# zdebruine/singlet

Hardware: AMD Instinct MI355X
Metric: ALS iterations/sec (1M cells x 30k genes, 5% nnz, k=50) (higher is better)
Workload: dtype f64

## Files before the change

singlet_amd/csrc/gen_acc_tiled.py:

```python
#!/usr/bin/env python3
import os
import sys

NS = 8
ER = [64 + i for i in range(NS)]
EX = [72 + 2 * i for i in range(NS)]
AD = [88 + j for j in range(8)]
W = [96 + 4 * j for j in range(8)]
ACC = 128
S_RP, S_XP, S_NS, S_ACC = 84, 86, 88, 91
S_TP = 92
TAB0, TAB1 = 52, 68
S_END = 100


def r2(b):
    return f"v[{b}:{b + 1}]"


class Gen:

    def __init__(self, pair, pf=0):
        self.L = []
        self.lab = 0
        self.pair = pair
        self.pf = pf

    def A(self, s):
        self.L.append(s)

    def label(self, stem):
        self.lab += 1
        return f".Ltiled_{stem}_{self.lab}_%="

    def text(self):
        return " \\\n".join(f'    "{ins}\\n\\t"' for ins in self.L)

    def refill(self, i):
        if self.pair:
            st, sub = i >> 1, i & 1
            ro, xo, lap_r = 256 * st + 64 * sub, 512 * st + 128 * sub, 128 * NS
        else:
            ro, xo, lap_r = 256 * i, 512 * i, 256 * NS
        A = self.A
        A(f"global_load_dword v{ER[i]}, %[voff4], s[{S_RP}:{S_RP + 1}] offset:{ro}")
        A(f"global_load_dwordx2 {r2(EX[i])}, %[voff8], s[{S_XP}:{S_XP + 1}] offset:{xo}")
        if i == NS - 1:
            A(f"s_add_u32 s{S_RP}, s{S_RP}, {lap_r}")
            A(f"s_addc_u32 s{S_RP + 1}, s{S_RP + 1}, 0")
            A(f"s_add_u32 s{S_XP}, s{S_XP}, {2 * lap_r}")
            A(f"s_addc_u32 s{S_XP + 1}, s{S_XP + 1}, 0")

    def addrs(self, slot, o):
        for j in range(8):
            self.A(f"v_add_u32_dpp v{AD[j]}, v{ER[slot]}, %[lane16] row_newbcast:{8 * o + j} row_mask:0xf bank_mask:0xf")

    def octet(self, d, o, reads):
        A = self.A
        x = EX[d]
        for g in range(2):
            gi = 4 * d + 2 * o + g
            A(f"s_bfe_u32 m0, s{TAB0 + gi // 2}, {hex((16 * (gi & 1)) | (16 << 16))}")
            A(f"s_waitcnt lgkmcnt({4 if reads else 4 - 4 * g})")
            for j in range(4 * g, 4 * g + 4):
                bc = f"row_newbcast:{8 * o + j} row_mask:0xf bank_mask:0xf"
                A(f"v_fmac_f64_dpp {r2(ACC)}, {r2(x)}, {r2(W[j])} {bc}")
                A(f"v_fmac_f64_dpp {r2(ACC + 2)}, {r2(x)}, {r2(W[j] + 2)} {bc}")
                if reads:
                    A(f"ds_read_b128 v[{W[j]}:{W[j] + 3}], v{AD[j]}")

    def wrap(self):
        A = self.A
        A("s_waitcnt lgkmcnt(0)")
        for w in range(8):
            A(f"s_mov_b64 s[{TAB0 + 2 * w}:{TAB0 + 2 * w + 1}], s[{TAB1 + 2 * w}:{TAB1 + 2 * w + 1}]")
        A(f"s_load_dwordx16 s[{TAB1}:{TAB1 + 15}], s[{S_TP}:{S_TP + 1}], 0x0")
        A(f"s_add_u32 s{S_TP}, s{S_TP}, 64")
        A(f"s_addc_u32 s{S_TP + 1}, s{S_TP + 1}, 0")
        if self.pf:
            A("s_mov_b32 m0, 0")
            A("v_lshlrev_b32 v63, 1, %[pfl]")
            A(f"global_load_dword v63, v63, s[{S_XP}:{S_XP + 1}]")
            A(f"global_load_dword v63, %[pfl], s[{S_RP}:{S_RP + 1}]")

    def body(self, d, L_body, L_last):
        A = self.A
        dn = (d + 1) % NS
        A(f"{L_body[d]}:")
        A("s_mov_b32 m0, 0")
        self.addrs(d, 1)
        self.octet(d, 0, True)
        A("s_mov_b32 m0, 0")
        A(f"s_waitcnt vmcnt({2 * (NS - 2) + (2 if (self.pf and d != NS - 1) else 0)})")
        self.addrs(dn, 0)
        self.octet(d, 1, True)
        self.refill(d)
        if d == NS - 1:
            self.wrap()
        A(f"s_sub_u32 s{S_NS}, s{S_NS}, 1")
        A(f"s_cbranch_scc1 {L_last[dn]}")
        if d == NS - 1:
            A(f"s_branch {L_body[0]}")

    def last(self, d, L_last, L_end):
        A = self.A
        A(f"{L_last[d]}:")
        A("s_mov_b32 m0, 0")
        self.addrs(d, 1)
        self.octet(d, 0, True)
        self.octet(d, 1, False)
        self.refill(d)
        A(f"s_mov_b32 %[phase], {(d + 1) % NS}")
        A(f"s_branch {L_end}")

    def chunk(self):
        A = self.A
        L_body = [self.label(f"b{d}") for d in range(NS)]
        L_pro = [self.label(f"p{d}") for d in range(NS)]
        L_last = [self.label(f"last{d}") for d in range(NS)]
        L_end = self.label("end")
        A(f"s_mov_b64 s[{S_RP}:{S_RP + 1}], %[rp]")
        A(f"s_mov_b64 s[{S_XP}:{S_XP + 1}], %[xp]")
        A(f"s_sub_u32 s{S_NS}, %[ns], 2")
        A(f"s_lshl_b32 s{S_ACC}, %[phase], 3")
        A(f"s_mov_b64 s[{S_TP}:{S_TP + 1}], %[tp]")
        A(f"s_sub_u32 s{S_TP}, s{S_TP}, s{S_ACC}")
        A(f"s_subb_u32 s{S_TP + 1}, s{S_TP + 1}, 0")
        A(f"s_load_dwordx16 s[{TAB0}:{TAB0 + 15}], s[{S_TP}:{S_TP + 1}], 0x0")
        A(f"s_load_dwordx16 s[{TAB1}:{TAB1 + 15}], s[{S_TP}:{S_TP + 1}], 0x40")
        A(f"s_add_u32 s{S_TP}, s{S_TP}, 128")
        A(f"s_addc_u32 s{S_TP + 1}, s{S_TP + 1}, 0")
        A(f"s_mov_b32 s{S_ACC}, 0")
        A(f"s_set_gpr_idx_on s{S_ACC}, 0")
        A("s_mov_b32 m0, 0")
        for d in range(1, NS):
            A(f"s_cmp_eq_u32 %[phase], {d}")
            A(f"s_cbranch_scc1 {L_pro[d]}")
        for d in range(NS):
            A(f"{L_pro[d]}:")
            A(f"s_waitcnt vmcnt({2 * (NS - 1)})")
            self.addrs(d, 0)
            for j in range(8):
                A(f"ds_read_b128 v[{W[j]}:{W[j] + 3}], v{AD[j]}")
            A("s_waitcnt lgkmcnt(0)")
            A(f"s_cmp_eq_u32 %[ns], 1")
            A(f"s_cbranch_scc1 {L_last[d]}")
            A(f"s_branch {L_body[d]}")
        for d in range(NS):
            self.body(d, L_body, L_last)
        for d in range(NS):
            self.last(d, L_last, L_end)
        A(f"{L_end}:")
        A("s_waitcnt lgkmcnt(0)")
        A("s_mov_b32 m0, 0")
        A("s_set_gpr_idx_off")
        A(f"s_mov_b64 %[rp], s[{S_RP}:{S_RP + 1}]")
        A(f"s_mov_b64 %[xp], s[{S_XP}:{S_XP + 1}]")

    def ring_fill(self):
        A = self.A
        A(f"s_mov_b64 s[{S_RP}:{S_RP + 1}], %[rp]")
        A(f"s_mov_b64 s[{S_XP}:{S_XP + 1}], %[xp]")
        for i in range(NS):
            self.refill(i)
        A(f"s_mov_b64 %[rp], s[{S_RP}:{S_RP + 1}]")
        A(f"s_mov_b64 %[xp], s[{S_XP}:{S_XP + 1}]")


def main():
    pf = int(os.environ.get("SGL_GEN_PF", "0"))
    out = ["// generated by gen_acc_tiled.py -- do not edit", "#pragma once"]
    g = Gen(pair=False)
    for c in range(128):
        g.A(f"v_mov_b32 v{ACC + c}, 0")
    out.append(f"#define ACC_TILED_ZERO_ASM \\\n{g.text()}")
    out.append("#define ACC_TILED_CLOBBERS " + ", ".join([f'"s{r}"' for r in range(83, S_END)] + ['"memory"', '"scc"']))
    for tag, pair in (("2", True), ("4", False)):
        g = Gen(pair)
        g.ring_fill()
        out.append("")
        out.append(f"#define ACC_TILED{tag}_RING_FILL_ASM \\\n{g.text()}")
        g = Gen(pair, pf)
        g.chunk()
        out.append("")
        out.append(f"#define ACC_TILED{tag}_CHUNK_ASM \\\n{g.text()}")
    tclob = [f'"s{r}"' for r in range(TAB0, S_END)] + ['"memory"', '"scc"'] + (['"v63"'] if pf else [])
    out.append("#define ACC_TILED_CHUNK_CLOBBERS " + ", ".join(tclob))
    out.append(f"#define ACC_TILED_PF_LAPS {pf}")
    sys.stdout.write("\n".join(out) + "\n")


if __name__ == "__main__":
    main()
```

singlet_amd/csrc/kernels_tiled.hip:

```cpp
#include "sgl_internal.h"
#include <hipcub/hipcub.hpp>
#include <stdlib.h>
#include <utility>
#include <type_traits>

#define TILED_NW 8
#define TILED_CW 64
#define TILED_NP 32
#define TILED_LDS_BYTES (160 * 1024 - 512)
#define TILED_SLACK 4096

__device__ __forceinline__ int64_t tiled_slot_col(const int32_t* __restrict__ perm, int64_t ncol, int64_t wb, int h, int p, int nsl) {
    const int64_t pos = wb * (TILED_NP * nsl) + nsl * p + h;
    if (pos >= ncol) return -1;
    return perm ? (int64_t)perm[pos] : pos;
}

__device__ __forceinline__ int tiled_ranges_of(int64_t wb, int R, int64_t tail_wg0, int tail_R) {
    return (tail_R > 1 && tail_wg0 >= 0 && wb / TILED_NW >= tail_wg0) ? tail_R : R;
}
__device__ __forceinline__ int tiled_range_end(int b, int T, int NB, int nr) {
    const int t = b >> 1;
    const int y = (int)(((int64_t)(t + 1) * nr - 1) / T);
    const int b1 = 2 * (int)(((int64_t)(y + 1) * T) / nr);
    return b1 < NB ? b1 : NB;
}

__global__ __launch_bounds__(256) void tiled_count_kernel(const int64_t* __restrict__ seg, const int32_t* __restrict__ perm, int64_t ncol,
                                                          int T, int NB, int64_t nwb, int R, int64_t tail_wg0, int tail_R,
                                                          uint8_t* __restrict__ cnt, uint16_t* __restrict__ ahead,
                                                          int64_t* __restrict__ chunk_entries, int nsl) {
    const int lane = threadIdx.x & 63, p = lane & 31;
    const int64_t wb = ((int64_t)blockIdx.x * blockDim.x + threadIdx.x) >> 6;
    if (wb >= nwb) return;
    const int gps = 16 / nsl;
    int64_t col[4];
    for (int h = 0; h < 4; ++h) col[h] = h < nsl ? tiled_slot_col(perm, ncol, wb, h, p, nsl) : -1;
    const int nr = tiled_ranges_of(wb, R, tail_wg0, tail_R);
    for (int b0 = 0; b0 < NB;) {
        const int b1 = tiled_range_end(b0, T, NB, nr);
        int64_t pos[4];
        for (int h = 0; h < 4; ++h) pos[h] = col[h] >= 0 ? seg[(int64_t)b0 * ncol + col[h]] : 0;
        for (int b = b0; b < b1; ++b) {
            const int hi = b + 2 < b1 ? b + 2 : b1;
            int64_t must = 0, avail = 0, ew[4];
            for (int h = 0; h < 4; ++h) {
                ew[h] = 0;
                if (col[h] >= 0) {
                    const int64_t eb = seg[(int64_t)(b + 1) * ncol + col[h]];
                    ew[h] = seg[(int64_t)hi * ncol + col[h]];
                    must = eb - pos[h] > must ? eb - pos[h] : must;
                    avail = ew[h] - pos[h] > avail ? ew[h] - pos[h] : avail;
                }
            }
            int g = (int)((must + 3) >> 2);
            const int cap = (int)((avail + 3) >> 2) - g;
            int tot = g;
            for (int o = 16; o > 0; o >>= 1) tot += __shfl_xor(tot, o, 32);
            const int rem = (gps - (tot & (gps - 1))) & (gps - 1);
            int suf = cap;
            for (int o = 1; o < 32; o <<= 1) {
                const int v = __shfl_down(suf, o, 32);
                if (p + o < 32) suf += v;
            }
            const int above = suf - cap;
            int extra = rem - above < cap ? rem - above : cap;
            if (extra < 0) extra = 0;
            const int all = __shfl(suf, 0, 32);
            if (p == TILED_NP - 1 && rem > all) extra += rem - all;
            g += extra;
            const int64_t u = wb * NB + b;
            if (lane < 32) {
                cnt[u * TILED_NP + p] = (uint8_t)g;
                for (int h = 0; h < nsl; ++h)
                    ahead[u * (TILED_NP * nsl) + nsl * p + h] = col[h] >= 0 ? (uint16_t)(pos[h] - seg[(int64_t)b * ncol + col[h]]) : (uint16_t)0;
            }
            if (lane == 0) chunk_entries[u] = (int64_t)(tot + rem) * 4 * nsl;
            for (int h = 0; h < 4; ++h) pos[h] += (4 * (int64_t)g < ew[h] - pos[h]) ? 4 * (int64_t)g : ew[h] - pos[h];
        }
        b0 = b1;
    }
}

__global__ __launch_bounds__(256) void tiled_fill_kernel(const double* __restrict__ x, const int32_t* __restrict__ idx,
                                                         const int64_t* __restrict__ seg, const int32_t* __restrict__ perm,
                                                         int64_t ncol, int T, int NB, int64_t nwb, int R, int64_t tail_wg0, int tail_R,
                                                         int D, int row_bytes, const uint8_t* __restrict__ cnt,
                                                         const uint16_t* __restrict__ ahead, const int64_t* __restrict__ cstart,
                                                         uint32_t* __restrict__ sroff, double* __restrict__ sx,
                                                         int masked, uint64_t seed, SglDiv inv_density, int mask_t,
                                                         int64_t col_off, int64_t row_off, int nsl) {
    const int lane = threadIdx.x & 63;
    const int eps = 64 / nsl, eps_sh = nsl == 4 ? 4 : 5;
    const int64_t gw = ((int64_t)blockIdx.x * blockDim.x + threadIdx.x) >> 6;
    const int64_t nw = ((int64_t)gridDim.x * blockDim.x) >> 6;
    for (int64_t u = gw; u < nwb * NB; u += nw) {
        const int64_t wb = u / NB;
        const int b = (int)(u - wb * NB);
        const int b1 = tiled_range_end(b, T, NB, tiled_ranges_of(wb, R, tail_wg0, tail_R));
        const int hi = b + 2 < b1 ? b + 2 : b1;
        const int64_t c0 = cstart[u];
        int P = 0;
        for (int p = 0; p < TILED_NP; ++p) {
            const int n4 = 4 * (int)cnt[u * TILED_NP + p];
            if (n4 == 0) continue;
            for (int h = 0; h < nsl; ++h) {
                const int64_t col = tiled_slot_col(perm, ncol, wb, h, p, nsl);
                int64_t a = 0, e = 0;
                if (col >= 0) {
                    a = seg[(int64_t)b * ncol + col] + ahead[u * (TILED_NP * nsl) + nsl * p + h];
                    e = seg[(int64_t)hi * ncol + col];
                }
                for (int q = lane; q < n4; q += 64) {
                    uint32_t ro = 0;
                    double xv = 0.0;
                    if (a + q < e) {
                        const int32_t r = idx[a + q];
                        const int blk = r >= (b + 1) * D ? b + 1 : b;
                        ro = (uint32_t)((blk & 1) * D + (r - blk * D)) * (uint32_t)row_bytes;
                        xv = x[a + q];
                        if (masked) {
                            const uint64_t gc = (uint64_t)(col + col_off), gr = (uint64_t)(r + row_off);
                            if (mask_t ? sgl_draw(seed, gr, gc, inv_density) : sgl_draw(seed, gc, gr, inv_density)) xv = 0.0;
                        }
                    }
                    const int pos = P + q;
                    const int64_t dst = c0 + (int64_t)(pos >> eps_sh) * 64 + h * eps + (pos & (eps - 1));
                    if (sroff != nullptr) sroff[dst] = ro;
                    sx[dst] = xv;
                }
            }
            P += n4;
        }
    }
}

__global__ __launch_bounds__(256) void tiled_gtab_kernel(const uint8_t* __restrict__ cnt, const int64_t* __restrict__ cstart,
                                                         int64_t nchunks, int nsl, uint16_t* __restrict__ gtab) {
    const int lane = threadIdx.x & 63;
    const int64_t gw = ((int64_t)blockIdx.x * blockDim.x + threadIdx.x) >> 6;
    const int64_t nw = ((int64_t)gridDim.x * blockDim.x) >> 6;
    for (int64_t u = gw; u < nchunks; u += nw) {
        int64_t g0 = cstart[u] / (4 * nsl);
        for (int p = 0; p < TILED_NP; ++p) {
            const int n = (int)cnt[u * TILED_NP + p];
            for (int q = lane; q < n; q += 64) gtab[g0 + q] = (uint16_t)(0x8000u | (unsigned)(4 * p));
            g0 += n;
        }
    }
}

template <typename T_>
static int t_alloc(T_** p, size_t count) {
    *p = nullptr;
    if (count == 0) count = 1;
    hipError_t e = sgl_pool_malloc((void**)p, count * sizeof(T_));
    if (e != hipSuccess) {
        (void)hipGetLastError();
        sgl_set_error("hipMalloc of %zu bytes failed: %s", count * sizeof(T_), hipGetErrorString(e));
        return SGL_ENOMEM;
    }
    return SGL_OK;
}

template <typename T_>
static int t_reserve(T_** p, size_t* cap, size_t count) {
    if (*p != nullptr && *cap >= count) return SGL_OK;
    if (*p) (void)sgl_pool_free(*p);
    *p = nullptr;
    *cap = 0;
    const size_t want = count + count / 32 + 64;
    SGLCHK(t_alloc(p, want));
    *cap = want;
    return SGL_OK;
}

void sgl_tiled_free(DevTiled& S) {
    if (S.seg) (void)sgl_pool_free(S.seg);
    if (S.perm) (void)sgl_pool_free(S.perm);
    if (S.roff) (void)sgl_pool_free(S.roff);
    if (S.x) (void)sgl_pool_free(S.x);
    if (S.cstart) (void)sgl_pool_free(S.cstart);
    if (S.cnt) (void)sgl_pool_free(S.cnt);
    if (S.ahead) (void)sgl_pool_free(S.ahead);
    if (S.gtab) (void)sgl_pool_free(S.gtab);
    if (S.part) (void)sgl_pool_free(S.part);
    if (S.xm) (void)sgl_pool_free(S.xm);
    S = DevTiled();
}

static bool tiled_sort_columns() {
    const char* e = getenv("SGL_TILED_SORT");
    return !(e && *e == '0');
}

__global__ void tiled_col_keys_kernel(const int64_t* __restrict__ p, int64_t ncol, uint32_t* __restrict__ keys, int32_t* __restrict__ iota) {
    for (int64_t c = (int64_t)blockIdx.x * blockDim.x + threadIdx.x; c < ncol; c += (int64_t)gridDim.x * blockDim.x) {
        keys[c] = (uint32_t)(p[c + 1] - p[c]);
        iota[c] = (int32_t)c;
    }
}

static int tiled_build_perm(sgl_ctx* c, const DevCSC& M, DevTiled& S) {
    hipStream_t s = c->stream;
    const int64_t n = M.ncol;
    SGLCHK(t_reserve(&S.perm, &S.cap_perm, (size_t)n));
    uint32_t *keys = nullptr, *keys_out = nullptr;
    int32_t* iota = nullptr;
    void* tmp = nullptr;
    int rc = t_alloc(&keys, (size_t)n);
    if (rc == SGL_OK) rc = t_alloc(&keys_out, (size_t)n);
    if (rc == SGL_OK) rc = t_alloc(&iota, (size_t)n);
    if (rc == SGL_OK && n > 0) {
        const int64_t blocks = std::min<int64_t>((n + 255) / 256, 4096);
        tiled_col_keys_kernel<<<dim3((unsigned)blocks), dim3(256), 0, s>>>(M.p, n, keys, iota);
        size_t tmp_bytes = 0;
        if (hipcub::DeviceRadixSort::SortPairsDescending(nullptr, tmp_bytes, keys, keys_out, iota, S.perm, n, 0, 32, s) != hipSuccess) rc = SGL_EHIP;
        if (rc == SGL_OK && sgl_pool_malloc(&tmp, tmp_bytes ? tmp_bytes : 1) != hipSuccess) { (void)hipGetLastError(); rc = SGL_ENOMEM; }
        if (rc == SGL_OK && hipcub::DeviceRadixSort::SortPairsDescending(tmp, tmp_bytes, keys, keys_out, iota, S.perm, n, 0, 32, s) != hipSuccess) rc = SGL_EHIP;
    }
    static_assert(TILED_CW == 64, "pair layout: 64 columns per wave");
    std::vector<uint32_t> top_v((size_t)TILED_NW * TILED_CW * 2);
    uint32_t* top = top_v.data();
    const int64_t ntop = std::min<int64_t>(n, (int64_t)top_v.size());
    if (rc == SGL_OK && ntop > 0 && hipMemcpyAsync(top, keys_out, sizeof(uint32_t) * (size_t)ntop, hipMemcpyDeviceToHost, s) != hipSuccess) rc = SGL_EHIP;
    const hipError_t e = hipStreamSynchronize(s);
    if (rc == SGL_OK && e == hipSuccess) {
        int64_t tn = 0, tn2 = 0;
        for (int64_t q = 0; q < ntop; ++q) {
            if (q < TILED_NW * TILED_CW) tn += top[q];
            tn2 += top[q];
        }
        S.top_share = M.nnz > 0 ? (double)tn / (double)M.nnz : 0.0;
        S.top_share4 = M.nnz > 0 ? (double)tn2 / (double)M.nnz : 0.0;
    }
    if (keys) (void)sgl_pool_free(keys);
    if (keys_out) (void)sgl_pool_free(keys_out);
    if (iota) (void)sgl_pool_free(iota);
    if (tmp) (void)sgl_pool_free(tmp);
    if (rc == SGL_OK && e != hipSuccess) rc = SGL_EHIP;
    if (rc != SGL_OK) { sgl_set_error("tiled build: sorting the columns by their non-zero count failed"); return rc; }
    S.perm_nnz = M.nnz;
    return SGL_OK;
}

void sgl_trace_setup(const char* what);

int sgl_tiled_build(sgl_ctx* c, const DevCSC& M, int k, DevTiled& S) {
    hipStream_t s = c->stream;
    const int nsl = (k <= 32 && !getenv("SGL_TILED_NO_QUAD")) ? 4 : 2;
    if (S.built && S.k == k && S.NSL == nsl && S.ncol == M.ncol && S.nrow == M.nrow && S.src_nnz == M.nnz && (S.perm != nullptr) == tiled_sort_columns())
        return SGL_OK;
    S.built = false;
    S.xm_mask_t = -1;
    S.k = k;
    S.NSL = nsl;
    S.CW = TILED_NP * nsl;
    const int KS = nsl == 4 ? 32 : ((k + 1) & ~1);
    S.KS = KS;
    int TR = TILED_LDS_BYTES / (KS * 8);
    TR = TR / 8 * 8;
    if (TR > 984) TR = 984;
    if (TR < 8 || k > 64) { sgl_set_error("tiled accumulate: k=%d unsupported", k); return SGL_EINVAL; }
    S.nwb = ((int64_t)M.ncol + S.CW - 1) / S.CW;
    {
        const int64_t groups = (S.nwb + TILED_NW - 1) / TILED_NW, T0 = ((int64_t)M.nrow + TR - 1) / TR;
        if (groups * T0 < 256 && !getenv("SGL_TILED_FULL_TILES")) {
            const int64_t want = std::min<int64_t>((256 + groups - 1) / groups, ((int64_t)M.nrow + 127) / 128);
            if (want > T0) TR = std::min<int>(TR, (int)(((((int64_t)M.nrow + want - 1) / want) + 7) / 8 * 8));
        }
    }
    S.TR = TR;
    S.T = (int)((M.nrow + TR - 1) / TR);
    const int D = TR / 2;
    S.NB = (int)((M.nrow + D - 1) / D);
    S.ncol = M.ncol;
    S.nrow = M.nrow;
    S.src_nnz = M.nnz;
    const int64_t nchunks = S.nwb * S.NB;

    int rc = SGL_OK;
    if (!tiled_sort_columns()) {
        if (S.perm) { (void)sgl_pool_free(S.perm); S.perm = nullptr; S.cap_perm = 0; }
    } else if (!S.perm || S.perm_nnz != M.nnz || S.cap_perm < (size_t)M.ncol) {
        rc = tiled_build_perm(c, M, S);
    }
    sgl_trace_setup("  stream: column order");
    const double E_est = (double)M.nnz * 1.06;
    const int64_t nwg_x = (S.nwb + TILED_NW - 1) / TILED_NW;
    int R = 1;
    const int r_fill = nwg_x < 1024 ? (int)std::max<int64_t>(1, (512 + nwg_x - 1) / nwg_x) : 1;
    const double top_share = nsl == 4 ? S.top_share4 : S.top_share;
    const bool skewed = S.perm && top_share * (double)nwg_x > 1.5;
    const int r_bal = skewed ? (int)std::min<double>(256.0, ceil(top_share * 256.0 / 0.35)) : 1;
    if (r_bal > r_fill) {
        double best = -1.0;
        const int rmin = std::max(r_fill, (int)std::min<int64_t>(r_bal, std::max(1, S.T)));
        if (rmin > S.T) R = std::max(1, S.T);
        for (int r = rmin; r <= std::min<int64_t>(S.T, rmin + rmin / 4 + 4); ++r) {
            const int tpr = (S.T + r - 1) / r;
            const int reff = (S.T + tpr - 1) / tpr;
            const double wgs = (double)nwg_x * reff;
            const double eff = wgs / (ceil(wgs / 256.0) * 256.0);
            if (eff > best + 1e-9) { best = eff; R = reff; }
        }
    } else if (r_fill > 1 && S.T > 1) {
        const double t_tile = E_est / (double)nsl / ((double)nwg_x * (double)S.T) * 2.4e-9 + 2.5e-6;
        const double t_wg = 6e-6;
        double best = 1e300;
        for (int r = 1; r <= std::min<int64_t>(S.T, 64); ++r) {
            const double wgs = (double)nwg_x * r;
            const double rounds = ceil(wgs / 256.0);
            const int largest = (S.T + r - 1) / r;
            const double cost = rounds * ((double)largest * t_tile + t_wg) + (r > 1 ? (double)r * (double)k * (double)M.ncol * 16.0 / 4e12 : 0.0);
            if (cost < best * (1.0 - 1e-9)) { best = cost; R = r; }
        }
    }
    if (const char* fr = getenv("SGL_TILED_RANGES")) {
        if (atoi(fr) > 0) R = atoi(fr);
    }
    S.range_fastest = r_bal > r_fill;
    S.R = std::max(1, std::min(R, std::max(1, S.T)));
    S.tiles_per_range = (S.T + S.R - 1) / S.R;
    S.tail_wg0 = -1;
    S.tail_R = 1;
    if (S.R == 1 && !S.range_fastest && nwg_x > 256 && S.T > 1 && E_est >= (double)(4ll << 20) && !getenv("SGL_TILED_NO_TAIL")) {
        const int64_t tail = nwg_x % 256;
        if (tail > 0) {
            const double t_tile = E_est / (double)nsl / ((double)nwg_x * (double)S.T) * 2.4e-9 + 2.5e-6;
            const double t_wg = 6e-6;
            const double tail_cols = (double)tail * TILED_NW * S.CW;
            double best = (double)S.T * t_tile + t_wg;
            int Rt = 1;
            for (int r = 2; r <= std::min<int64_t>(S.T, 16); ++r) {
                const double rounds = ceil((double)tail * r / 256.0);
                const double cost = rounds * ((double)((S.T + r - 1) / r) * t_tile + t_wg) + (double)r * (double)k * tail_cols * 16.0 / 4e12;
                if (cost < best * (1.0 - 1e-9)) { best = cost; Rt = r; }
            }
            if (Rt > 1) { S.tail_wg0 = nwg_x - tail; S.tail_R = Rt; }
        }
    }
    if (rc == SGL_OK) rc = t_reserve(&S.seg, &S.cap_seg, (size_t)(S.NB + 1) * (size_t)M.ncol);
    sgl_trace_setup("  stream: segment buffer reserved");
    DevCSC tmp = M;
    tmp.tile_rows = D;
    tmp.ntiles = S.NB;
    tmp.seg = S.seg;
    if (rc == SGL_OK) rc = k_build_segments(s, tmp);
    int64_t* chunk_entries = nullptr;
    if (rc == SGL_OK) rc = t_alloc(&chunk_entries, (size_t)nchunks);
    if (rc == SGL_OK) rc = t_reserve(&S.cnt, &S.cap_cnt, (size_t)nchunks * TILED_NP);
    if (rc == SGL_OK) rc = t_reserve(&S.ahead, &S.cap_ahead, (size_t)nchunks * (size_t)S.CW);
    if (rc == SGL_OK) rc = t_reserve(&S.cstart, &S.cap_cstart, (size_t)nchunks + 1);
    if (rc == SGL_OK && S.nwb > 0) {
        tiled_count_kernel<<<dim3((unsigned)((S.nwb + 3) / 4)), dim3(256), 0, s>>>(S.seg, S.perm, M.ncol, S.T, S.NB, S.nwb, S.R,
                                                                                   S.tail_wg0, S.tail_R, S.cnt, S.ahead, chunk_entries, nsl);
        if (hipGetLastError() != hipSuccess) { sgl_set_error("tiled build: count kernel launch failed"); rc = SGL_EHIP; }
    }
    if (rc == SGL_OK) rc = k_exclusive_scan(c, chunk_entries, S.cstart, nchunks);
    if (rc == SGL_OK) rc = k_scan_total(s, chunk_entries, S.cstart, nchunks);
    int64_t E = 0;
    if (rc == SGL_OK) {
        if (hipMemcpyAsync(&E, S.cstart + nchunks, sizeof(int64_t), hipMemcpyDeviceToHost, s) != hipSuccess ||
            hipStreamSynchronize(s) != hipSuccess) { sgl_set_error("tiled build: reading the stream size failed"); rc = SGL_EHIP; }
    }
    S.E = E;
    sgl_trace_setup("  stream: segments, counts, scan");
    if (rc == SGL_OK) rc = t_reserve(&S.roff, &S.cap_roff, (size_t)E + TILED_SLACK);
    if (rc == SGL_OK) rc = t_reserve(&S.x, &S.cap_x, (size_t)E + TILED_SLACK);
    sgl_trace_setup("  stream: roff / x buffers reserved");
    if (rc == SGL_OK) {
        if (hipMemsetAsync(S.roff + E, 0, TILED_SLACK * sizeof(uint32_t), s) != hipSuccess ||
            hipMemsetAsync(S.x + E, 0, TILED_SLACK * sizeof(double), s) != hipSuccess) { sgl_set_error("tiled build: clearing the stream slack failed"); rc = SGL_EHIP; }
    }
    if (rc == SGL_OK && nchunks > 0) {
        int64_t blocks = (nchunks + 3) / 4;
        if (blocks > 256 * 64) blocks = 256 * 64;
        tiled_fill_kernel<<<dim3((unsigned)blocks), dim3(256), 0, s>>>(M.x, M.i, S.seg, S.perm, M.ncol, S.T, S.NB, S.nwb, S.R, S.tail_wg0,
                                                                       S.tail_R, D, KS * 8, S.cnt, S.ahead, S.cstart, S.roff, S.x,
                                                                       0, 0, sgl_div_make(1), 0, 0, 0, nsl);
        if (hipGetLastError() != hipSuccess) { sgl_set_error("tiled build: fill kernel launch failed"); rc = SGL_EHIP; }
    }
    const size_t ngroups = (size_t)(E / (4 * nsl));
    if (rc == SGL_OK) rc = t_reserve(&S.gtab, &S.cap_gtab, ngroups + 256);
    if (rc == SGL_OK) {
        if (hipMemsetAsync(S.gtab + ngroups, 0, 256 * sizeof(uint16_t), s) != hipSuccess) { sgl_set_error("tiled build: clearing the schedule slack failed"); rc = SGL_EHIP; }
    }
    if (rc == SGL_OK && nchunks > 0) {
        int64_t blocks = (nchunks + 3) / 4;
        if (blocks > 256 * 64) blocks = 256 * 64;
        tiled_gtab_kernel<<<dim3((unsigned)blocks), dim3(256), 0, s>>>(S.cnt, S.cstart, nchunks, nsl, S.gtab);
        if (hipGetLastError() != hipSuccess) { sgl_set_error("tiled build: schedule kernel launch failed"); rc = SGL_EHIP; }
    }
    if (rc == SGL_OK && S.R > 1) rc = t_reserve(&S.part, &S.cap_part, (size_t)S.R * (size_t)k * (size_t)M.ncol);
    if (rc == SGL_OK && S.tail_R > 1)
        rc = t_reserve(&S.part, &S.cap_part, (size_t)S.tail_R * (size_t)k * (size_t)((nwg_x - S.tail_wg0) * TILED_NW * S.CW));
    hipError_t e = hipStreamSynchronize(s);
    if (chunk_entries) (void)sgl_pool_free(chunk_entries);
    if (rc == SGL_OK && e != hipSuccess) { sgl_set_error("tiled build failed: %s", hipGetErrorString(e)); rc = SGL_EHIP; }
    if (rc != SGL_OK) { sgl_tiled_free(S); return rc; }
    S.built = true;
    ++S.builds;
    return rc;
}

int sgl_tiled_mask_values(sgl_ctx* c, const DevCSC& M, DevTiled& S, uint64_t seed, uint64_t inv_density, int mask_t,
                          int64_t col_off, int64_t row_off) {
    if (!S.built || !S.seg || !S.ahead) { sgl_set_error("masked values: no entry stream"); return SGL_ESTATE; }
    if (S.xm && S.xm_seed == seed && S.xm_inv == inv_density && S.xm_mask_t == mask_t) return SGL_OK;
    hipStream_t s = c->stream;
    S.xm_mask_t = -1;
    SGLCHK(t_reserve(&S.xm, &S.cap_xm, (size_t)S.E + TILED_SLACK));
    HIPCHK(hipMemsetAsync(S.xm + S.E, 0, TILED_SLACK * sizeof(double), s));
    const int64_t nchunks = S.nwb * S.NB;
    if (nchunks > 0) {
        const int KS = S.KS;
        int64_t blocks = (nchunks + 3) / 4;
        if (blocks > 256 * 64) blocks = 256 * 64;
        tiled_fill_kernel<<<dim3((unsigned)blocks), dim3(256), 0, s>>>(M.x, M.i, S.seg, S.perm, M.ncol, S.T, S.NB, S.nwb, S.R, S.tail_wg0,
                                                                       S.tail_R, S.TR / 2, KS * 8, S.cnt, S.ahead, S.cstart, nullptr, S.xm,
                                                                       1, seed, sgl_div_make(inv_density), mask_t, col_off, row_off, S.NSL);
        HIPCHK(hipGetLastError());
    }
    S.xm_seed = seed; S.xm_inv = inv_density; S.xm_mask_t = mask_t;
    return SGL_OK;
}


__device__ __forceinline__ void acc_load(int idx4, double& v0, double& v1) {
    int a, b, c, d;
    asm volatile(
        "s_set_gpr_idx_on %4, gpr_idx(SRC0)\n\tv_mov_b32 %0, v128\n\tv_mov_b32 %1, v129\n\tv_mov_b32 %2, v130\n\t"
        "v_mov_b32 %3, v131\n\ts_set_gpr_idx_off"
        : "=v"(a), "=v"(b), "=v"(c), "=v"(d) : "s"(idx4) : "memory");
    v0 = __hiloint2double(b, a);
    v1 = __hiloint2double(d, c);
}

#include "acc_tiled_gen.inc"

template <int NSL>
__device__ __forceinline__ void tiled_stage(double* __restrict__ tile, const double* __restrict__ src, int rows, int k, int KS, int ldf,
                                            bool sync) {
    const int n = rows * k;
    if constexpr (NSL == 4) {
        const int c16 = (int)threadIdx.x & 15, r0 = (int)threadIdx.x >> 4;
        constexpr int RPR = 64 * TILED_NW / 16;
        const bool vec = ((k | ldf) & 1) == 0 && (reinterpret_cast<uintptr_t>(src) & 15) == 0;
        if (vec) {
            constexpr int RST = 4;
            double2 stg[RST];
            const bool cact = 2 * c16 < k;
#pragma unroll
            for (int j = 0; j < RST; ++j) {
                const int r = r0 + j * RPR;
                stg[j] = double2{0.0, 0.0};
                if (cact && r < rows) stg[j] = *reinterpret_cast<const double2*>(src + (int64_t)r * ldf + 2 * c16);
            }
            if (sync) __syncthreads();
            for (int rb = 0; rb < rows; rb += RST * RPR) {
#pragma unroll
                for (int j = 0; j < RST; ++j) {
                    const int r = rb + r0 + j * RPR;
                    if (cact && r < rows) *reinterpret_cast<double2*>(tile + r * 32 + 2 * c16) = stg[j];
                }
                if (rb + RST * RPR < rows) {
#pragma unroll
                    for (int j = 0; j < RST; ++j) {
                        const int r = rb + RST * RPR + r0 + j * RPR;
                        stg[j] = double2{0.0, 0.0};
                        if (cact && r < rows) stg[j] = *reinterpret_cast<const double2*>(src + (int64_t)r * ldf + 2 * c16);
                    }
                }
            }
        } else {
            if (sync) __syncthreads();
            for (int r = r0; r < rows; r += RPR) {
                if (c16 < k) tile[r * 32 + c16] = src[(int64_t)r * ldf + c16];
                if (c16 + 16 < k) tile[r * 32 + c16 + 16] = src[(int64_t)r * ldf + c16 + 16];
            }
        }
    } else {
        if (sync) __syncthreads();
        if (((k | ldf) & 1) == 0 && (reinterpret_cast<uintptr_t>(src) & 15) == 0) {
            const int hp = k >> 1;
            for (int e = (int)threadIdx.x; e < rows * hp; e += 64 * TILED_NW) {
                const int r = e / hp, c2 = (e - r * hp) * 2;
                *reinterpret_cast<double2*>(tile + r * KS + c2) = *reinterpret_cast<const double2*>(src + (int64_t)r * ldf + c2);
            }
        } else {
            for (int e = (int)threadIdx.x; e < n; e += 64 * TILED_NW) {
                const int r = e / k, f = e - r * k;
                tile[r * KS + f] = src[(int64_t)r * ldf + f];
            }
        }
        if (KS != k)
            for (int r = (int)threadIdx.x; r < rows; r += 64 * TILED_NW) tile[r * KS + k] = 0.0;
    }
}

#define TILED_PIECES 10
static_assert(TILED_PIECES * 64 * TILED_NW * 16 >= TILED_LDS_BYTES / 2, "the pieces must cover a whole ring slot");
#define TILED_PIECE_CLOBBERS "v24", "v25", "v26", "v27", "v28", "v29", "v30", "v31", "v32", "v33", "v34", "v35", "v36", "v37", "v38", \
    "v39", "v40", "v41", "v42", "v43", "v44", "v45", "v46", "v47", "v48", "v49", "v50", "v51", "v52", "v53", "v54", "v55", "v56", "v57", \
    "v58", "v59", "v60", "v61", "v62", "v63"

#define TILED_ISSUE_PIECE(regs, off) \
    "v_add_u32 %[t], " off ", %[o]\n\tv_min_u32 %[t], %[last], %[t]\n\tglobal_load_dwordx4 " regs ", %[t], %[src]\n\t"

__device__ __forceinline__ void tiled_issue(const double* src, int n) {
    static_assert(TILED_PIECES == 10, "tiled_issue / tiled_commit move ten pieces");
    const unsigned o = threadIdx.x * 16u, last = (unsigned)n * 8u - 16u;
    unsigned t;
    asm volatile(
        "v_min_u32 %[t], %[last], %[o]\n\tglobal_load_dwordx4 v[24:27], %[t], %[src]\n\t"
        TILED_ISSUE_PIECE("v[28:31]", "0x2000") TILED_ISSUE_PIECE("v[32:35]", "0x4000") TILED_ISSUE_PIECE("v[36:39]", "0x6000")
        TILED_ISSUE_PIECE("v[40:43]", "0x8000") TILED_ISSUE_PIECE("v[44:47]", "0xa000") TILED_ISSUE_PIECE("v[48:51]", "0xc000")
        TILED_ISSUE_PIECE("v[52:55]", "0xe000") TILED_ISSUE_PIECE("v[56:59]", "0x10000") TILED_ISSUE_PIECE("v[60:63]", "0x12000")
        : [t] "=&v"(t)
        : [o] "v"(o), [last] "s"(last), [src] "s"(src)
        : TILED_PIECE_CLOBBERS);
}

#define TILED_COMMIT_PIECE(regs, addr, off) \
    "v_cmp_gt_i32 vcc, %[lim], %[a]\n\ts_and_b64 exec, exec, vcc\n\tds_write_b128 " addr ", " regs off "\n\ts_sub_i32 %[lim], %[lim], 0x2000\n\t"
#define TILED_COMMIT_ASM(wait) \
    "s_waitcnt vmcnt(" wait ")\n\ts_mov_b64 %[sv], exec\n\t" \
    TILED_COMMIT_PIECE("v[24:27]", "%[a]", "") TILED_COMMIT_PIECE("v[28:31]", "%[a]", " offset:8192") \
    TILED_COMMIT_PIECE("v[32:35]", "%[a]", " offset:16384") TILED_COMMIT_PIECE("v[36:39]", "%[a]", " offset:24576") \
    TILED_COMMIT_PIECE("v[40:43]", "%[a]", " offset:32768") TILED_COMMIT_PIECE("v[44:47]", "%[a]", " offset:40960") \
    TILED_COMMIT_PIECE("v[48:51]", "%[a]", " offset:49152") TILED_COMMIT_PIECE("v[52:55]", "%[a]", " offset:57344") \
    TILED_COMMIT_PIECE("v[56:59]", "%[a1]", "") TILED_COMMIT_PIECE("v[60:63]", "%[a1]", " offset:8192") \
    "s_mov_b64 exec, %[sv]\n\ts_waitcnt lgkmcnt(0)"
#define TILED_COMMIT_OPERANDS : [sv] "=&s"(sv), [lim] "+s"(lim) : [a] "v"(a), [a1] "v"(a + 65536u) : "vcc", "scc", "memory"

__device__ __forceinline__ void tiled_commit(double* tile, int n, bool ring_after) {
    typedef __attribute__((address_space(3))) char lds_char;
    const unsigned base = (unsigned)(uintptr_t)(lds_char*)tile;
    const unsigned a = base + threadIdx.x * 16u;
    int lim = (int)(base + (unsigned)n * 8u);
    uint64_t sv;
    if (ring_after)
        asm volatile(TILED_COMMIT_ASM("16") TILED_COMMIT_OPERANDS);
    else
        asm volatile(TILED_COMMIT_ASM("0") TILED_COMMIT_OPERANDS);
}

#define ACC_TILED_PARAMS                                                                                                          \
    const uint32_t* __restrict__ sroff, const double* __restrict__ sx, const int64_t* __restrict__ cstart,                            \
        const uint8_t* __restrict__ cnt, int T, int NB, int64_t nwb, const double* __restrict__ F, int k, int TR, int64_t nrow,       \
        int tiles_per_range, double* __restrict__ Bout, int64_t ncol, int KS, int ldf, int ldb, int64_t slab,                        \
        const int32_t* __restrict__ perm, int range_fastest, const uint16_t* __restrict__ gtab, int tail_wg0, int tail_R,            \
        double* __restrict__ tail_part, int64_t tail_slab
#define ACC_TILED_ARGS \
    sroff, sx, cstart, cnt, T, NB, nwb, F, k, TR, nrow, tiles_per_range, Bout, ncol, KS, ldf, ldb, slab, perm, range_fastest, gtab, \
        tail_wg0, tail_R, tail_part, tail_slab
template <int NSL>
__device__ __forceinline__ void acc_tiled_body(ACC_TILED_PARAMS) {
    asm volatile("" ::: "v255");
    extern __shared__ __attribute__((aligned(16))) char smem[];
    double* tile = reinterpret_cast<double*>(smem);
    const int lane = threadIdx.x & 63;
    const int wave = __builtin_amdgcn_readfirstlane((int)(threadIdx.x >> 6));
    unsigned bx = blockIdx.x, by = blockIdx.y;
    if (range_fastest) {
        const unsigned unit = blockIdx.x + gridDim.x * blockIdx.y, nranges = gridDim.y;
        bx = unit / nranges;
        by = unit - bx * nranges;
    }
    unsigned nry = gridDim.y;
    bool tail_piece = false;
    if (tail_R > 1 && (int)bx >= tail_wg0) {
        const unsigned u = bx - (unsigned)tail_wg0;
        bx = (unsigned)tail_wg0 + u / (unsigned)tail_R;
        by = u % (unsigned)tail_R;
        nry = (unsigned)tail_R;
        tail_piece = true;
    }
    const int64_t wb = (int64_t)bx * TILED_NW + wave;
    const int t0 = (int)(((int64_t)by * T) / nry);
    const int t1 = (int)((((int64_t)by + 1) * T) / nry);
    const int D = TR >> 1;
    const int b0 = 2 * t0, b1 = 2 * t1 < NB ? 2 * t1 : NB;
    const bool wact = wb < nwb;
    typedef __attribute__((address_space(3))) char lds_char;
    constexpr int LMASK = NSL == 4 ? 15 : 31;
    const unsigned lane16 = (unsigned)(uintptr_t)(lds_char*)smem + (lane & LMASK) * 16;
    const unsigned slot = NSL == 2 ? (unsigned)((lane >> 5) * 32 + (lane & 15)) : (unsigned)lane;
    const unsigned voff4 = slot * 4, voff8 = slot * 8;
    constexpr unsigned LAP_R = (NSL == 4 ? 256u : 128u) * 8u;
    const unsigned pfl = (unsigned)lane * (LAP_R / 64u) + (unsigned)ACC_TILED_PF_LAPS * LAP_R;

    asm volatile(ACC_TILED_ZERO_ASM ::: "memory");

    uint64_t rp = 0, xp = 0;
    int phase = 0;
    int64_t pos_next = 0;
    if (wact) {
        const int64_t pos = cstart[wb * NB + b0];
        pos_next = cstart[wb * NB + b0 + 1];
        const uint64_t r_ = reinterpret_cast<uint64_t>(sroff + pos), x_ = reinterpret_cast<uint64_t>(sx + pos);
        rp = ((uint64_t)(uint32_t)__builtin_amdgcn_readfirstlane((unsigned)(r_ >> 32)) << 32) | (uint32_t)__builtin_amdgcn_readfirstlane((unsigned)r_);
        xp = ((uint64_t)(uint32_t)__builtin_amdgcn_readfirstlane((unsigned)(x_ >> 32)) << 32) | (uint32_t)__builtin_amdgcn_readfirstlane((unsigned)x_);
        if constexpr (NSL == 4)
            asm volatile(ACC_TILED4_RING_FILL_ASM : [rp] "+s"(rp), [xp] "+s"(xp) : [voff4] "v"(voff4), [voff8] "v"(voff8) : ACC_TILED_CLOBBERS);
        else
            asm volatile(ACC_TILED2_RING_FILL_ASM : [rp] "+s"(rp), [xp] "+s"(xp) : [voff4] "v"(voff4), [voff8] "v"(voff8) : ACC_TILED_CLOBBERS);
    }
    if constexpr (NSL == 4) {
        for (int e = (int)threadIdx.x; e < TILED_LDS_BYTES / 8; e += 64 * TILED_NW) tile[e] = 0.0;
    }

    const bool pf = NSL == 2 && KS == k && ldf == k;
    auto block_rows = [&](int j) { const int64_t row0 = (int64_t)j * D; return (int)(nrow - row0 < D ? nrow - row0 : D); };
    int64_t pos_cur = wact ? cstart[wb * NB + b0] : 0;
    for (int b = b0; b < b1; ++b) {
        const int nsets = (int)((pos_next - pos_cur) >> 6);
        const int64_t pos_chunk = pos_cur;
        pos_cur = pos_next;
        if (wact && b + 1 < b1) pos_next = cstart[wb * NB + b + 2];

        if (pf) {
            if (b == b0) {
#pragma clang loop unroll(disable)
                for (int j = b; j <= b + 1 && j < b1; ++j) {
                    tiled_issue(F + (int64_t)j * D * ldf, block_rows(j) * k);
                    tiled_commit(tile + (j & 1) * D * KS, block_rows(j) * k, false);
                }
                __syncthreads();
            }
            if (b + 2 < b1) tiled_issue(F + (int64_t)(b + 2) * D * ldf, block_rows(b + 2) * k);
        } else {
#pragma clang loop unroll(disable)
            for (int j = b == b0 ? b : b + 1; j <= b + 1 && j < b1; ++j) {
                const int64_t row0 = (int64_t)j * D;
                tiled_stage<NSL>(tile + (j & 1) * D * KS, F + row0 * ldf, block_rows(j), k, KS, ldf, j == b || b != b0);
            }
            if (b == b0 || b + 1 < b1) {
                __builtin_amdgcn_s_waitcnt(0x0F70);
                __syncthreads();
            }
        }
        if (wact && nsets > 0) {
            const uint64_t t_ = reinterpret_cast<uint64_t>(gtab + pos_chunk / (4 * NSL));
            const uint64_t tp = ((uint64_t)(uint32_t)__builtin_amdgcn_readfirstlane((unsigned)(t_ >> 32)) << 32) | (uint32_t)__builtin_amdgcn_readfirstlane((unsigned)t_);
            if constexpr (NSL == 2)
                asm volatile(ACC_TILED2_CHUNK_ASM
                             : [rp] "+s"(rp), [xp] "+s"(xp), [phase] "+s"(phase)
                             : [ns] "s"(2 * nsets), [tp] "s"(tp), [lane16] "v"(lane16), [voff4] "v"(voff4), [voff8] "v"(voff8), [pfl] "v"(pfl)
                             : ACC_TILED_CHUNK_CLOBBERS);
            else
                asm volatile(ACC_TILED4_CHUNK_ASM
                             : [rp] "+s"(rp), [xp] "+s"(xp), [phase] "+s"(phase)
                             : [ns] "s"(nsets), [tp] "s"(tp), [lane16] "v"(lane16), [voff4] "v"(voff4), [voff8] "v"(voff8), [pfl] "v"(pfl)
                             : ACC_TILED_CHUNK_CLOBBERS);
        }
        if (pf && b + 2 < b1) {
            __syncthreads();
            tiled_commit(tile + (b & 1) * D * KS, block_rows(b + 2) * k, wact && nsets >= 4);
            __syncthreads();
        }
    }
    asm volatile("s_waitcnt vmcnt(0)" ::: "memory");
    if (wact) {
        double* out = Bout + (size_t)by * (size_t)slab;
        const int f = 2 * (lane & LMASK);
        const int64_t tail_pos0 = (int64_t)tail_wg0 * TILED_NW * (TILED_NP * NSL);
        for (int p = 0; p < TILED_NP; ++p) {
            double v0, v1;
            acc_load(4 * p, v0, v1);
            const int h = NSL == 4 ? (lane >> 4) : (lane >> 5);
            const int64_t col = tiled_slot_col(perm, ncol, wb, h, p, NSL);
            if (col >= 0) {
                if (tail_piece) {
                    const int64_t pos = wb * (TILED_NP * NSL) + NSL * p + h;
                    double* o = tail_part + (size_t)by * (size_t)tail_slab + (pos - tail_pos0) * k;
                    if (f < k) o[f] = v0;
                    if (f + 1 < k) o[f + 1] = v1;
                } else {
                    if (f < k) out[col * ldb + f] = v0;
                    if (f + 1 < k) out[col * ldb + f + 1] = v1;
                }
            }
        }
    }
}

template <int NSL>
__global__ __launch_bounds__(512) __attribute__((amdgpu_waves_per_eu(8, 8))) void acc_tiled_kernel(ACC_TILED_PARAMS) {
    acc_tiled_body<NSL>(ACC_TILED_ARGS);
}
template <>
__global__ __launch_bounds__(512) __attribute__((amdgpu_waves_per_eu(8, 8), amdgpu_num_vgpr(12))) void acc_tiled_kernel<2>(ACC_TILED_PARAMS) {
    acc_tiled_body<2>(ACC_TILED_ARGS);
}

__global__ void acc_tiled_reduce_kernel(const double* __restrict__ part, int R, int64_t n, int k, int ldb, double* __restrict__ B) {
    for (int64_t e = (int64_t)blockIdx.x * blockDim.x + threadIdx.x; e < n; e += (int64_t)gridDim.x * blockDim.x) {
        double s = part[e];
        for (int r = 1; r < R; ++r) s += part[(size_t)r * n + e];
        if (ldb == k) {
            B[e] = s;
        } else {
            const int64_t col = e / k;
            B[col * ldb + (e - col * k)] = s;
        }
    }
}

__global__ void acc_tiled_reduce_tail_kernel(const double* __restrict__ part, int R, int64_t slab, int64_t pos0, int64_t ncol,
                                             const int32_t* __restrict__ perm, int k, int ldb, double* __restrict__ B) {
    const int64_t n = (ncol - pos0) * k;
    for (int64_t e = (int64_t)blockIdx.x * blockDim.x + threadIdx.x; e < n; e += (int64_t)gridDim.x * blockDim.x) {
        double s = part[e];
        for (int r = 1; r < R; ++r) s += part[(size_t)r * slab + e];
        const int64_t q = e / k;
        const int64_t col = perm ? (int64_t)perm[pos0 + q] : pos0 + q;
        B[col * ldb + (e - q * k)] = s;
    }
}

int k_acc_tiled(hipStream_t s, const DevTiled& S, const double* F, int ldf, double* B, int ldb, int kf, const double* xvals) {
    if (S.ncol <= 0) return SGL_OK;
    if (kf <= 0 || kf > S.k) { sgl_set_error("k_acc_tiled: bad part size %d (stream built for %d)", kf, S.k); return SGL_EINVAL; }
    const int KS = S.KS;
    const size_t lds = S.NSL == 4 ? (size_t)TILED_LDS_BYTES + 512 : (size_t)S.TR * KS * 8 + 512;
    SGLCHK(sgl_allow_dynamic_lds<&acc_tiled_kernel<2>>(TILED_LDS_BYTES + 512));
    SGLCHK(sgl_allow_dynamic_lds<&acc_tiled_kernel<4>>(TILED_LDS_BYTES + 512));
    const int64_t nwg_x = (S.nwb + TILED_NW - 1) / TILED_NW;
    const bool slabs = S.R > 1;
    double* out = slabs ? S.part : B;
    const int64_t n = (int64_t)kf * S.ncol;
    const bool tail = !slabs && S.tail_R > 1 && S.tail_wg0 >= 0;
    const int64_t tail_cols = tail ? (nwg_x - S.tail_wg0) * TILED_NW * S.CW : 0;
    const int64_t tail_slab = tail_cols * kf;
    const dim3 grid(tail ? (unsigned)(S.tail_wg0 + (nwg_x - S.tail_wg0) * S.tail_R) : (unsigned)nwg_x, (unsigned)S.R);
    auto launch = [&](auto nsl) {
        acc_tiled_kernel<decltype(nsl)::value><<<grid, dim3(64 * TILED_NW), lds, s>>>(
            S.roff, xvals ? xvals : S.x, S.cstart, S.cnt, S.T, S.NB, S.nwb, F, kf, S.TR, S.nrow, S.tiles_per_range, out, S.ncol, KS, ldf,
            slabs ? kf : ldb, slabs ? n : 0, S.perm, S.range_fastest ? 1 : 0, S.gtab, tail ? (int)S.tail_wg0 : -1, tail ? S.tail_R : 1,
            S.part, tail_slab);
    };
    if (S.NSL == 4) launch(std::integral_constant<int, 4>());
    else launch(std::integral_constant<int, 2>());
    HIPCHK(hipGetLastError());
    if (tail) {
        const int64_t pos0 = S.tail_wg0 * TILED_NW * S.CW;
        const int64_t ne = (S.ncol - pos0) * kf;
        if (ne > 0) {
            int64_t blocks = (ne + 255) / 256;
            if (blocks > 4096) blocks = 4096;
            acc_tiled_reduce_tail_kernel<<<dim3((unsigned)blocks), dim3(256), 0, s>>>(S.part, S.tail_R, tail_slab, pos0, S.ncol, S.perm, kf, ldb, B);
            HIPCHK(hipGetLastError());
        }
    }
    if (slabs) {
        int64_t blocks = (n + 255) / 256;
        if (blocks > 4096) blocks = 4096;
        acc_tiled_reduce_kernel<<<dim3((unsigned)blocks), dim3(256), 0, s>>>(S.part, S.R, n, kf, ldb, B);
        HIPCHK(hipGetLastError());
    }
    return SGL_OK;
}

int k_acc_tiled_all(hipStream_t s, const DevTiled& S, const double* F, double* B, int k, const double* xvals) {
    for (int f0 = 0; f0 < k; f0 += S.k) {
        const int kf = (k - f0 < S.k) ? (k - f0) : S.k;
        SGLCHK(k_acc_tiled(s, S, F + f0, k, B + f0, k, kf, xvals));
    }
    return SGL_OK;
}

int tiled_part_size(int k) {
    if (k <= 64) return k;
    if (k > SGL_MAX_K) return 0;
    const bool quad = !getenv("SGL_TILED_NO_QUAD");
    const int parts = quad ? (k <= 96 ? 3 : (k + 31) / 32) : (k + 63) / 64;
    return ((k + parts - 1) / parts + 1) & ~1;
}
```

Before: 42.12.

## Add late-entry chunk variant that overlaps factor-tile prefetch with first ring lap

Adds a second generated chunk assembly variant for the NSL=2 prefetch path. Its first lap uses vmcnt thresholds that account for the ten outstanding tiled_issue factor-tile loads, so the sparse ring loop can start before those loads finish instead of waiting for them. The kernel body moves into a shared header and is compiled into a separate late kernel, which is selected by default when the prefetch conditions hold. The cost is more code size, extra branches in the first lap, and an environment switch to fall back.

```diff
diff --git a/singlet_amd/csrc/acc_tiled_body.h b/singlet_amd/csrc/acc_tiled_body.h
--- /dev/null
+++ b/singlet_amd/csrc/acc_tiled_body.h
@@ -0,0 +1,286 @@
+#pragma once
+#include "sgl_internal.h"
+
+#define TILED_NW 8
+#define TILED_CW 64
+#define TILED_NP 32
+#define TILED_LDS_BYTES (160 * 1024 - 512)
+#define TILED_SLACK 4096
+
+__device__ __forceinline__ int64_t tiled_slot_col(const int32_t* __restrict__ perm, int64_t ncol, int64_t wb, int h, int p, int nsl) {
+    const int64_t pos = wb * (TILED_NP * nsl) + nsl * p + h;
+    if (pos >= ncol) return -1;
+    return perm ? (int64_t)perm[pos] : pos;
+}
+
+
+__device__ __forceinline__ void acc_load(int idx4, double& v0, double& v1) {
+    int a, b, c, d;
+    asm volatile(
+        "s_set_gpr_idx_on %4, gpr_idx(SRC0)\n\tv_mov_b32 %0, v128\n\tv_mov_b32 %1, v129\n\tv_mov_b32 %2, v130\n\t"
+        "v_mov_b32 %3, v131\n\ts_set_gpr_idx_off"
+        : "=v"(a), "=v"(b), "=v"(c), "=v"(d) : "s"(idx4) : "memory");
+    v0 = __hiloint2double(b, a);
+    v1 = __hiloint2double(d, c);
+}
+
+#include "acc_tiled_gen.inc"
+
+template <int NSL>
+__device__ __forceinline__ void tiled_stage(double* __restrict__ tile, const double* __restrict__ src, int rows, int k, int KS, int ldf,
+                                            bool sync) {
+    const int n = rows * k;
+    if constexpr (NSL == 4) {
+        const int c16 = (int)threadIdx.x & 15, r0 = (int)threadIdx.x >> 4;
+        constexpr int RPR = 64 * TILED_NW / 16;
+        const bool vec = ((k | ldf) & 1) == 0 && (reinterpret_cast<uintptr_t>(src) & 15) == 0;
+        if (vec) {
+            constexpr int RST = 4;
+            double2 stg[RST];
+            const bool cact = 2 * c16 < k;
+#pragma unroll
+            for (int j = 0; j < RST; ++j) {
+                const int r = r0 + j * RPR;
+                stg[j] = double2{0.0, 0.0};
+                if (cact && r < rows) stg[j] = *reinterpret_cast<const double2*>(src + (int64_t)r * ldf + 2 * c16);
+            }
+            if (sync) __syncthreads();
+            for (int rb = 0; rb < rows; rb += RST * RPR) {
+#pragma unroll
+                for (int j = 0; j < RST; ++j) {
+                    const int r = rb + r0 + j * RPR;
+                    if (cact && r < rows) *reinterpret_cast<double2*>(tile + r * 32 + 2 * c16) = stg[j];
+                }
+                if (rb + RST * RPR < rows) {
+#pragma unroll
+                    for (int j = 0; j < RST; ++j) {
+                        const int r = rb + RST * RPR + r0 + j * RPR;
+                        stg[j] = double2{0.0, 0.0};
+                        if (cact && r < rows) stg[j] = *reinterpret_cast<const double2*>(src + (int64_t)r * ldf + 2 * c16);
+                    }
+                }
+            }
+        } else {
+            if (sync) __syncthreads();
+            for (int r = r0; r < rows; r += RPR) {
+                if (c16 < k) tile[r * 32 + c16] = src[(int64_t)r * ldf + c16];
+                if (c16 + 16 < k) tile[r * 32 + c16 + 16] = src[(int64_t)r * ldf + c16 + 16];
+            }
+        }
+    } else {
+        if (sync) __syncthreads();
+        if (((k | ldf) & 1) == 0 && (reinterpret_cast<uintptr_t>(src) & 15) == 0) {
+            const int hp = k >> 1;
+            for (int e = (int)threadIdx.x; e < rows * hp; e += 64 * TILED_NW) {
+                const int r = e / hp, c2 = (e - r * hp) * 2;
+                *reinterpret_cast<double2*>(tile + r * KS + c2) = *reinterpret_cast<const double2*>(src + (int64_t)r * ldf + c2);
+            }
+        } else {
+            for (int e = (int)threadIdx.x; e < n; e += 64 * TILED_NW) {
+                const int r = e / k, f = e - r * k;
+                tile[r * KS + f] = src[(int64_t)r * ldf + f];
+            }
+        }
+        if (KS != k)
+            for (int r = (int)threadIdx.x; r < rows; r += 64 * TILED_NW) tile[r * KS + k] = 0.0;
+    }
+}
+
+#define TILED_PIECES 10
+static_assert(TILED_PIECES * 64 * TILED_NW * 16 >= TILED_LDS_BYTES / 2, "the pieces must cover a whole ring slot");
+#define TILED_PIECE_CLOBBERS "v24", "v25", "v26", "v27", "v28", "v29", "v30", "v31", "v32", "v33", "v34", "v35", "v36", "v37", "v38", \
+    "v39", "v40", "v41", "v42", "v43", "v44", "v45", "v46", "v47", "v48", "v49", "v50", "v51", "v52", "v53", "v54", "v55", "v56", "v57", \
+    "v58", "v59", "v60", "v61", "v62", "v63"
+
+#define TILED_ISSUE_PIECE(regs, off) \
+    "v_add_u32 %[t], " off ", %[o]\n\tv_min_u32 %[t], %[last], %[t]\n\tglobal_load_dwordx4 " regs ", %[t], %[src]\n\t"
+
+__device__ __forceinline__ void tiled_issue(const double* src, int n) {
+    static_assert(TILED_PIECES == 10, "tiled_issue / tiled_commit move ten pieces");
+    const unsigned o = threadIdx.x * 16u, last = (unsigned)n * 8u - 16u;
+    unsigned t;
+    asm volatile(
+        "v_min_u32 %[t], %[last], %[o]\n\tglobal_load_dwordx4 v[24:27], %[t], %[src]\n\t"
+        TILED_ISSUE_PIECE("v[28:31]", "0x2000") TILED_ISSUE_PIECE("v[32:35]", "0x4000") TILED_ISSUE_PIECE("v[36:39]", "0x6000")
+        TILED_ISSUE_PIECE("v[40:43]", "0x8000") TILED_ISSUE_PIECE("v[44:47]", "0xa000") TILED_ISSUE_PIECE("v[48:51]", "0xc000")
+        TILED_ISSUE_PIECE("v[52:55]", "0xe000") TILED_ISSUE_PIECE("v[56:59]", "0x10000") TILED_ISSUE_PIECE("v[60:63]", "0x12000")
+        : [t] "=&v"(t)
+        : [o] "v"(o), [last] "s"(last), [src] "s"(src)
+        : TILED_PIECE_CLOBBERS);
+}
+
+#define TILED_COMMIT_PIECE(regs, addr, off) \
+    "v_cmp_gt_i32 vcc, %[lim], %[a]\n\ts_and_b64 exec, exec, vcc\n\tds_write_b128 " addr ", " regs off "\n\ts_sub_i32 %[lim], %[lim], 0x2000\n\t"
+#define TILED_COMMIT_ASM(wait) \
+    "s_waitcnt vmcnt(" wait ")\n\ts_mov_b64 %[sv], exec\n\t" \
+    TILED_COMMIT_PIECE("v[24:27]", "%[a]", "") TILED_COMMIT_PIECE("v[28:31]", "%[a]", " offset:8192") \
+    TILED_COMMIT_PIECE("v[32:35]", "%[a]", " offset:16384") TILED_COMMIT_PIECE("v[36:39]", "%[a]", " offset:24576") \
+    TILED_COMMIT_PIECE("v[40:43]", "%[a]", " offset:32768") TILED_COMMIT_PIECE("v[44:47]", "%[a]", " offset:40960") \
+    TILED_COMMIT_PIECE("v[48:51]", "%[a]", " offset:49152") TILED_COMMIT_PIECE("v[52:55]", "%[a]", " offset:57344") \
+    TILED_COMMIT_PIECE("v[56:59]", "%[a1]", "") TILED_COMMIT_PIECE("v[60:63]", "%[a1]", " offset:8192") \
+    "s_mov_b64 exec, %[sv]\n\ts_waitcnt lgkmcnt(0)"
+#define TILED_COMMIT_OPERANDS : [sv] "=&s"(sv), [lim] "+s"(lim) : [a] "v"(a), [a1] "v"(a + 65536u) : "vcc", "scc", "memory"
+
+__device__ __forceinline__ void tiled_commit(double* tile, int n, bool ring_after) {
+    typedef __attribute__((address_space(3))) char lds_char;
+    const unsigned base = (unsigned)(uintptr_t)(lds_char*)tile;
+    const unsigned a = base + threadIdx.x * 16u;
+    int lim = (int)(base + (unsigned)n * 8u);
+    uint64_t sv;
+    if (ring_after)
+        asm volatile(TILED_COMMIT_ASM("16") TILED_COMMIT_OPERANDS);
+    else
+        asm volatile(TILED_COMMIT_ASM("0") TILED_COMMIT_OPERANDS);
+}
+
+#define ACC_TILED_PARAMS                                                                                                          \
+    const uint32_t* __restrict__ sroff, const double* __restrict__ sx, const int64_t* __restrict__ cstart,                            \
+        const uint8_t* __restrict__ cnt, int T, int NB, int64_t nwb, const double* __restrict__ F, int k, int TR, int64_t nrow,       \
+        int tiles_per_range, double* __restrict__ Bout, int64_t ncol, int KS, int ldf, int ldb, int64_t slab,                        \
+        const int32_t* __restrict__ perm, int range_fastest, const uint16_t* __restrict__ gtab, int tail_wg0, int tail_R,            \
+        double* __restrict__ tail_part, int64_t tail_slab
+#define ACC_TILED_ARGS \
+    sroff, sx, cstart, cnt, T, NB, nwb, F, k, TR, nrow, tiles_per_range, Bout, ncol, KS, ldf, ldb, slab, perm, range_fastest, gtab, \
+        tail_wg0, tail_R, tail_part, tail_slab
+template <int NSL>
+__device__ __forceinline__ void acc_tiled_body(ACC_TILED_PARAMS) {
+    asm volatile("" ::: "v255");
+    extern __shared__ __attribute__((aligned(16))) char smem[];
+    double* tile = reinterpret_cast<double*>(smem);
+    const int lane = threadIdx.x & 63;
+    const int wave = __builtin_amdgcn_readfirstlane((int)(threadIdx.x >> 6));
+    unsigned bx = blockIdx.x, by = blockIdx.y;
+    if (range_fastest) {
+        const unsigned unit = blockIdx.x + gridDim.x * blockIdx.y, nranges = gridDim.y;
+        bx = unit / nranges;
+        by = unit - bx * nranges;
+    }
+    unsigned nry = gridDim.y;
+    bool tail_piece = false;
+    if (tail_R > 1 && (int)bx >= tail_wg0) {
+        const unsigned u = bx - (unsigned)tail_wg0;
+        bx = (unsigned)tail_wg0 + u / (unsigned)tail_R;
+        by = u % (unsigned)tail_R;
+        nry = (unsigned)tail_R;
+        tail_piece = true;
+    }
+    const int64_t wb = (int64_t)bx * TILED_NW + wave;
+    const int t0 = (int)(((int64_t)by * T) / nry);
+    const int t1 = (int)((((int64_t)by + 1) * T) / nry);
+    const int D = TR >> 1;
+    const int b0 = 2 * t0, b1 = 2 * t1 < NB ? 2 * t1 : NB;
+    const bool wact = wb < nwb;
+    typedef __attribute__((address_space(3))) char lds_char;
+    constexpr int LMASK = NSL == 4 ? 15 : 31;
+    const unsigned lane16 = (unsigned)(uintptr_t)(lds_char*)smem + (lane & LMASK) * 16;
+    const unsigned slot = NSL == 2 ? (unsigned)((lane >> 5) * 32 + (lane & 15)) : (unsigned)lane;
+    const unsigned voff4 = slot * 4, voff8 = slot * 8;
+    constexpr unsigned LAP_R = (NSL == 4 ? 256u : 128u) * 8u;
+    const unsigned pfl = (unsigned)lane * (LAP_R / 64u) + (unsigned)ACC_TILED_PF_LAPS * LAP_R;
+
+    asm volatile(ACC_TILED_ZERO_ASM ::: "memory");
+
+    uint64_t rp = 0, xp = 0;
+    int phase = 0;
+    int64_t pos_next = 0;
+    if (wact) {
+        const int64_t pos = cstart[wb * NB + b0];
+        pos_next = cstart[wb * NB + b0 + 1];
+        const uint64_t r_ = reinterpret_cast<uint64_t>(sroff + pos), x_ = reinterpret_cast<uint64_t>(sx + pos);
+        rp = ((uint64_t)(uint32_t)__builtin_amdgcn_readfirstlane((unsigned)(r_ >> 32)) << 32) | (uint32_t)__builtin_amdgcn_readfirstlane((unsigned)r_);
+        xp = ((uint64_t)(uint32_t)__builtin_amdgcn_readfirstlane((unsigned)(x_ >> 32)) << 32) | (uint32_t)__builtin_amdgcn_readfirstlane((unsigned)x_);
+        if constexpr (NSL == 4)
+            asm volatile(ACC_TILED4_RING_FILL_ASM : [rp] "+s"(rp), [xp] "+s"(xp) : [voff4] "v"(voff4), [voff8] "v"(voff8) : ACC_TILED_CLOBBERS);
+        else
+            asm volatile(ACC_TILED2_RING_FILL_ASM : [rp] "+s"(rp), [xp] "+s"(xp) : [voff4] "v"(voff4), [voff8] "v"(voff8) : ACC_TILED_CLOBBERS);
+    }
+    if constexpr (NSL == 4) {
+        for (int e = (int)threadIdx.x; e < TILED_LDS_BYTES / 8; e += 64 * TILED_NW) tile[e] = 0.0;
+    }
+
+    const bool pf = NSL == 2 && KS == k && ldf == k;
+    auto block_rows = [&](int j) { const int64_t row0 = (int64_t)j * D; return (int)(nrow - row0 < D ? nrow - row0 : D); };
+    int64_t pos_cur = wact ? cstart[wb * NB + b0] : 0;
+    for (int b = b0; b < b1; ++b) {
+        const int nsets = (int)((pos_next - pos_cur) >> 6);
+        const int64_t pos_chunk = pos_cur;
+        pos_cur = pos_next;
+        if (wact && b + 1 < b1) pos_next = cstart[wb * NB + b + 2];
+
+        if (pf) {
+            if (b == b0) {
+#pragma clang loop unroll(disable)
+                for (int j = b; j <= b + 1 && j < b1; ++j) {
+                    tiled_issue(F + (int64_t)j * D * ldf, block_rows(j) * k);
+                    tiled_commit(tile + (j & 1) * D * KS, block_rows(j) * k, false);
+                }
+                __syncthreads();
+            }
+            if (b + 2 < b1) tiled_issue(F + (int64_t)(b + 2) * D * ldf, block_rows(b + 2) * k);
+        } else {
+#pragma clang loop unroll(disable)
+            for (int j = b == b0 ? b : b + 1; j <= b + 1 && j < b1; ++j) {
+                const int64_t row0 = (int64_t)j * D;
+                tiled_stage<NSL>(tile + (j & 1) * D * KS, F + row0 * ldf, block_rows(j), k, KS, ldf, j == b || b != b0);
+            }
+            if (b == b0 || b + 1 < b1) {
+                __builtin_amdgcn_s_waitcnt(0x0F70);
+                __syncthreads();
+            }
+        }
+        if (wact && nsets > 0) {
+            const uint64_t t_ = reinterpret_cast<uint64_t>(gtab + pos_chunk / (4 * NSL));
+            const uint64_t tp = ((uint64_t)(uint32_t)__builtin_amdgcn_readfirstlane((unsigned)(t_ >> 32)) << 32) | (uint32_t)__builtin_amdgcn_readfirstlane((unsigned)t_);
+            if constexpr (NSL == 2) {
+#ifdef ACC_TILED2_LATE_CHUNK_ASM
+                static_assert(ACC_TILED_LATE_PIECES == TILED_PIECES, "the first-lap counts are for tiled_issue's pieces");
+                const int late = __builtin_amdgcn_readfirstlane((ACC_TILED_LATE_ENTRY && pf && b != b0 && b + 2 < b1) ? 1 : 0);
+                asm volatile(ACC_TILED2_LATE_CHUNK_ASM
+                             : [rp] "+s"(rp), [xp] "+s"(xp), [phase] "+s"(phase)
+                             : [ns] "s"(2 * nsets), [tp] "s"(tp), [lane16] "v"(lane16), [voff4] "v"(voff4), [voff8] "v"(voff8), [pfl] "v"(pfl),
+                               [late] "s"(late)
+                             : ACC_TILED_CHUNK_CLOBBERS);
+#else
+                asm volatile(ACC_TILED2_CHUNK_ASM
+                             : [rp] "+s"(rp), [xp] "+s"(xp), [phase] "+s"(phase)
+                             : [ns] "s"(2 * nsets), [tp] "s"(tp), [lane16] "v"(lane16), [voff4] "v"(voff4), [voff8] "v"(voff8), [pfl] "v"(pfl)
+                             : ACC_TILED_CHUNK_CLOBBERS);
+#endif
+            } else
+                asm volatile(ACC_TILED4_CHUNK_ASM
+                             : [rp] "+s"(rp), [xp] "+s"(xp), [phase] "+s"(phase)
+                             : [ns] "s"(nsets), [tp] "s"(tp), [lane16] "v"(lane16), [voff4] "v"(voff4), [voff8] "v"(voff8), [pfl] "v"(pfl)
+                             : ACC_TILED_CHUNK_CLOBBERS);
+        }
+        if (pf && b + 2 < b1) {
+            __syncthreads();
+            tiled_commit(tile + (b & 1) * D * KS, block_rows(b + 2) * k, wact && nsets >= 4);
+            __syncthreads();
+        }
+    }
+    asm volatile("s_waitcnt vmcnt(0)" ::: "memory");
+    if (wact) {
+        double* out = Bout + (size_t)by * (size_t)slab;
+        const int f = 2 * (lane & LMASK);
+        const int64_t tail_pos0 = (int64_t)tail_wg0 * TILED_NW * (TILED_NP * NSL);
+        for (int p = 0; p < TILED_NP; ++p) {
+            double v0, v1;
+            acc_load(4 * p, v0, v1);
+            const int h = NSL == 4 ? (lane >> 4) : (lane >> 5);
+            const int64_t col = tiled_slot_col(perm, ncol, wb, h, p, NSL);
+            if (col >= 0) {
+                if (tail_piece) {
+                    const int64_t pos = wb * (TILED_NP * NSL) + NSL * p + h;
+                    double* o = tail_part + (size_t)by * (size_t)tail_slab + (pos - tail_pos0) * k;
+                    if (f < k) o[f] = v0;
+                    if (f + 1 < k) o[f + 1] = v1;
+                } else {
+                    if (f < k) out[col * ldb + f] = v0;
+                    if (f + 1 < k) out[col * ldb + f + 1] = v1;
+                }
+            }
+        }
+    }
+}
+
+int k_acc_tiled_late_launch(hipStream_t s, dim3 grid, size_t lds, ACC_TILED_PARAMS);
diff --git a/singlet_amd/csrc/gen_acc_tiled.py b/singlet_amd/csrc/gen_acc_tiled.py
--- a/singlet_amd/csrc/gen_acc_tiled.py
+++ b/singlet_amd/csrc/gen_acc_tiled.py
@@ -11,6 +11,7 @@
 S_RP, S_XP, S_NS, S_ACC = 84, 86, 88, 91
 S_TP = 92
 TAB0, TAB1 = 52, 68
+LATE_PIECES = 10
 S_END = 100
 
 
@@ -20,11 +21,12 @@
 
 class Gen:
 
-    def __init__(self, pair, pf=0):
+    def __init__(self, pair, pf=0, late=False):
         self.L = []
         self.lab = 0
         self.pair = pair
         self.pf = pf
+        self.late = late and not pf
 
     def A(self, s):
         self.L.append(s)
@@ -83,15 +85,16 @@
             A(f"global_load_dword v63, v63, s[{S_XP}:{S_XP + 1}]")
             A(f"global_load_dword v63, %[pfl], s[{S_RP}:{S_RP + 1}]")
 
-    def body(self, d, L_body, L_last):
+    def body(self, d, L_body, L_last, L_first=None):
         A = self.A
         dn = (d + 1) % NS
-        A(f"{L_body[d]}:")
+        first = L_first is not None
+        A(f"{(L_first if first else L_body)[d]}:")
         A("s_mov_b32 m0, 0")
         self.addrs(d, 1)
         self.octet(d, 0, True)
         A("s_mov_b32 m0, 0")
-        A(f"s_waitcnt vmcnt({2 * (NS - 2) + (2 if (self.pf and d != NS - 1) else 0)})")
+        A(f"s_waitcnt vmcnt({2 * (NS - 2) + (2 if (self.pf and d != NS - 1) else 0) + (LATE_PIECES if first else 0)})")
         self.addrs(dn, 0)
         self.octet(d, 1, True)
         self.refill(d)
@@ -99,8 +102,38 @@
             self.wrap()
         A(f"s_sub_u32 s{S_NS}, s{S_NS}, 1")
         A(f"s_cbranch_scc1 {L_last[dn]}")
-        if d == NS - 1:
+        if first:
+            A(f"s_cmp_eq_u32 %[phase], {(d + 2) % NS}")
+            A(f"s_cbranch_scc1 {L_body[dn]}")
+            if d == NS - 1:
+                A(f"s_branch {L_first[0]}")
+        elif d == NS - 1:
             A(f"s_branch {L_body[0]}")
+
+    def prologue(self, d, label, L_next, L_last, extra=0):
+        A = self.A
+        A(f"{label}:")
+        A(f"s_waitcnt vmcnt({2 * (NS - 1) + extra})")
+        self.addrs(d, 0)
+        for j in range(8):
+            A(f"ds_read_b128 v[{W[j]}:{W[j] + 3}], v{AD[j]}")
+        A("s_waitcnt lgkmcnt(0)")
+        A(f"s_cmp_eq_u32 %[ns], 1")
+        A(f"s_cbranch_scc1 {L_last[d]}")
+        A(f"s_branch {L_next[d]}")
+
+    def first_lap(self, L_fdisp, L_body, L_last):
+        A = self.A
+        L_fpro = [self.label(f"fp{d}") for d in range(NS)]
+        L_first = [self.label(f"f{d}") for d in range(NS)]
+        A(f"{L_fdisp}:")
+        for d in range(1, NS):
+            A(f"s_cmp_eq_u32 %[phase], {d}")
+            A(f"s_cbranch_scc1 {L_fpro[d]}")
+        for d in range(NS):
+            self.prologue(d, L_fpro[d], L_first, L_last, LATE_PIECES)
+        for d in range(NS):
+            self.body(d, L_body, L_last, L_first)
 
     def last(self, d, L_last, L_end):
         A = self.A
@@ -133,23 +166,21 @@
         A(f"s_mov_b32 s{S_ACC}, 0")
         A(f"s_set_gpr_idx_on s{S_ACC}, 0")
         A("s_mov_b32 m0, 0")
+        if self.late:
+            L_fdisp = self.label("fdisp")
+            A("s_cmp_eq_u32 %[late], 0")
+            A(f"s_cbranch_scc0 {L_fdisp}")
         for d in range(1, NS):
             A(f"s_cmp_eq_u32 %[phase], {d}")
             A(f"s_cbranch_scc1 {L_pro[d]}")
         for d in range(NS):
-            A(f"{L_pro[d]}:")
-            A(f"s_waitcnt vmcnt({2 * (NS - 1)})")
-            self.addrs(d, 0)
-            for j in range(8):
-                A(f"ds_read_b128 v[{W[j]}:{W[j] + 3}], v{AD[j]}")
-            A("s_waitcnt lgkmcnt(0)")
-            A(f"s_cmp_eq_u32 %[ns], 1")
-            A(f"s_cbranch_scc1 {L_last[d]}")
-            A(f"s_branch {L_body[d]}")
+            self.prologue(d, L_pro[d], L_body, L_last)
         for d in range(NS):
             self.body(d, L_body, L_last)
         for d in range(NS):
             self.last(d, L_last, L_end)
+        if self.late:
+            self.first_lap(L_fdisp, L_body, L_last)
         A(f"{L_end}:")
         A("s_waitcnt lgkmcnt(0)")
         A("s_mov_b32 m0, 0")
@@ -167,8 +198,19 @@
         A(f"s_mov_b64 %[xp], s[{S_XP}:{S_XP + 1}]")
 
 
+def main_late(pf):
+    g = Gen(True, pf, late=True)
+    g.chunk()
+    out = ["// generated by gen_acc_tiled.py --late-pieces -- do not edit", "#pragma once", "",
+           f"#define ACC_TILED2_LATE_CHUNK_ASM \\\n{g.text()}", f"#define ACC_TILED_LATE_PIECES {LATE_PIECES}",
+           f"#define ACC_TILED_LATE_ENTRY {1 if g.late else 0}"]
+    sys.stdout.write("\n".join(out) + "\n")
+
+
 def main():
     pf = int(os.environ.get("SGL_GEN_PF", "0"))
+    if sys.argv[1:] == ["--late-pieces"]:
+        return main_late(pf)
     out = ["// generated by gen_acc_tiled.py -- do not edit", "#pragma once"]
     g = Gen(pair=False)
     for c in range(128):
diff --git a/singlet_amd/csrc/kernels_tiled.hip b/singlet_amd/csrc/kernels_tiled.hip
--- a/singlet_amd/csrc/kernels_tiled.hip
+++ b/singlet_amd/csrc/kernels_tiled.hip
@@ -4,17 +4,8 @@
 #include <utility>
 #include <type_traits>
 
-#define TILED_NW 8
-#define TILED_CW 64
-#define TILED_NP 32
-#define TILED_LDS_BYTES (160 * 1024 - 512)
-#define TILED_SLACK 4096
-
-__device__ __forceinline__ int64_t tiled_slot_col(const int32_t* __restrict__ perm, int64_t ncol, int64_t wb, int h, int p, int nsl) {
-    const int64_t pos = wb * (TILED_NP * nsl) + nsl * p + h;
-    if (pos >= ncol) return -1;
-    return perm ? (int64_t)perm[pos] : pos;
-}
+#include "acc_tiled_body.h"
+
 
 __device__ __forceinline__ int tiled_ranges_of(int64_t wb, int R, int64_t tail_wg0, int tail_R) {
     return (tail_R > 1 && tail_wg0 >= 0 && wb / TILED_NW >= tail_wg0) ? tail_R : R;
@@ -427,265 +418,6 @@
 }
 
 
-__device__ __forceinline__ void acc_load(int idx4, double& v0, double& v1) {
-    int a, b, c, d;
-    asm volatile(
-        "s_set_gpr_idx_on %4, gpr_idx(SRC0)\n\tv_mov_b32 %0, v128\n\tv_mov_b32 %1, v129\n\tv_mov_b32 %2, v130\n\t"
-        "v_mov_b32 %3, v131\n\ts_set_gpr_idx_off"
-        : "=v"(a), "=v"(b), "=v"(c), "=v"(d) : "s"(idx4) : "memory");
-    v0 = __hiloint2double(b, a);
-    v1 = __hiloint2double(d, c);
-}
-
-#include "acc_tiled_gen.inc"
-
-template <int NSL>
-__device__ __forceinline__ void tiled_stage(double* __restrict__ tile, const double* __restrict__ src, int rows, int k, int KS, int ldf,
-                                            bool sync) {
-    const int n = rows * k;
-    if constexpr (NSL == 4) {
-        const int c16 = (int)threadIdx.x & 15, r0 = (int)threadIdx.x >> 4;
-        constexpr int RPR = 64 * TILED_NW / 16;
-        const bool vec = ((k | ldf) & 1) == 0 && (reinterpret_cast<uintptr_t>(src) & 15) == 0;
-        if (vec) {
-            constexpr int RST = 4;
-            double2 stg[RST];
-            const bool cact = 2 * c16 < k;
-#pragma unroll
-            for (int j = 0; j < RST; ++j) {
-                const int r = r0 + j * RPR;
-                stg[j] = double2{0.0, 0.0};
-                if (cact && r < rows) stg[j] = *reinterpret_cast<const double2*>(src + (int64_t)r * ldf + 2 * c16);
-            }
-            if (sync) __syncthreads();
-            for (int rb = 0; rb < rows; rb += RST * RPR) {
-#pragma unroll
-                for (int j = 0; j < RST; ++j) {
-                    const int r = rb + r0 + j * RPR;
-                    if (cact && r < rows) *reinterpret_cast<double2*>(tile + r * 32 + 2 * c16) = stg[j];
-                }
-                if (rb + RST * RPR < rows) {
-#pragma unroll
-                    for (int j = 0; j < RST; ++j) {
-                        const int r = rb + RST * RPR + r0 + j * RPR;
-                        stg[j] = double2{0.0, 0.0};
-                        if (cact && r < rows) stg[j] = *reinterpret_cast<const double2*>(src + (int64_t)r * ldf + 2 * c16);
-                    }
-                }
-            }
-        } else {
-            if (sync) __syncthreads();
-            for (int r = r0; r < rows; r += RPR) {
-                if (c16 < k) tile[r * 32 + c16] = src[(int64_t)r * ldf + c16];
-                if (c16 + 16 < k) tile[r * 32 + c16 + 16] = src[(int64_t)r * ldf + c16 + 16];
-            }
-        }
-    } else {
-        if (sync) __syncthreads();
-        if (((k | ldf) & 1) == 0 && (reinterpret_cast<uintptr_t>(src) & 15) == 0) {
-            const int hp = k >> 1;
-            for (int e = (int)threadIdx.x; e < rows * hp; e += 64 * TILED_NW) {
-                const int r = e / hp, c2 = (e - r * hp) * 2;
-                *reinterpret_cast<double2*>(tile + r * KS + c2) = *reinterpret_cast<const double2*>(src + (int64_t)r * ldf + c2);
-            }
-        } else {
-            for (int e = (int)threadIdx.x; e < n; e += 64 * TILED_NW) {
-                const int r = e / k, f = e - r * k;
-                tile[r * KS + f] = src[(int64_t)r * ldf + f];
-            }
-        }
-        if (KS != k)
-            for (int r = (int)threadIdx.x; r < rows; r += 64 * TILED_NW) tile[r * KS + k] = 0.0;
-    }
-}
-
-#define TILED_PIECES 10
-static_assert(TILED_PIECES * 64 * TILED_NW * 16 >= TILED_LDS_BYTES / 2, "the pieces must cover a whole ring slot");
-#define TILED_PIECE_CLOBBERS "v24", "v25", "v26", "v27", "v28", "v29", "v30", "v31", "v32", "v33", "v34", "v35", "v36", "v37", "v38", \
-    "v39", "v40", "v41", "v42", "v43", "v44", "v45", "v46", "v47", "v48", "v49", "v50", "v51", "v52", "v53", "v54", "v55", "v56", "v57", \
-    "v58", "v59", "v60", "v61", "v62", "v63"
-
-#define TILED_ISSUE_PIECE(regs, off) \
-    "v_add_u32 %[t], " off ", %[o]\n\tv_min_u32 %[t], %[last], %[t]\n\tglobal_load_dwordx4 " regs ", %[t], %[src]\n\t"
-
-__device__ __forceinline__ void tiled_issue(const double* src, int n) {
-    static_assert(TILED_PIECES == 10, "tiled_issue / tiled_commit move ten pieces");
-    const unsigned o = threadIdx.x * 16u, last = (unsigned)n * 8u - 16u;
-    unsigned t;
-    asm volatile(
-        "v_min_u32 %[t], %[last], %[o]\n\tglobal_load_dwordx4 v[24:27], %[t], %[src]\n\t"
-        TILED_ISSUE_PIECE("v[28:31]", "0x2000") TILED_ISSUE_PIECE("v[32:35]", "0x4000") TILED_ISSUE_PIECE("v[36:39]", "0x6000")
-        TILED_ISSUE_PIECE("v[40:43]", "0x8000") TILED_ISSUE_PIECE("v[44:47]", "0xa000") TILED_ISSUE_PIECE("v[48:51]", "0xc000")
-        TILED_ISSUE_PIECE("v[52:55]", "0xe000") TILED_ISSUE_PIECE("v[56:59]", "0x10000") TILED_ISSUE_PIECE("v[60:63]", "0x12000")
-        : [t] "=&v"(t)
-        : [o] "v"(o), [last] "s"(last), [src] "s"(src)
-        : TILED_PIECE_CLOBBERS);
-}
-
-#define TILED_COMMIT_PIECE(regs, addr, off) \
-    "v_cmp_gt_i32 vcc, %[lim], %[a]\n\ts_and_b64 exec, exec, vcc\n\tds_write_b128 " addr ", " regs off "\n\ts_sub_i32 %[lim], %[lim], 0x2000\n\t"
-#define TILED_COMMIT_ASM(wait) \
-    "s_waitcnt vmcnt(" wait ")\n\ts_mov_b64 %[sv], exec\n\t" \
-    TILED_COMMIT_PIECE("v[24:27]", "%[a]", "") TILED_COMMIT_PIECE("v[28:31]", "%[a]", " offset:8192") \
-    TILED_COMMIT_PIECE("v[32:35]", "%[a]", " offset:16384") TILED_COMMIT_PIECE("v[36:39]", "%[a]", " offset:24576") \
-    TILED_COMMIT_PIECE("v[40:43]", "%[a]", " offset:32768") TILED_COMMIT_PIECE("v[44:47]", "%[a]", " offset:40960") \
-    TILED_COMMIT_PIECE("v[48:51]", "%[a]", " offset:49152") TILED_COMMIT_PIECE("v[52:55]", "%[a]", " offset:57344") \
-    TILED_COMMIT_PIECE("v[56:59]", "%[a1]", "") TILED_COMMIT_PIECE("v[60:63]", "%[a1]", " offset:8192") \
-    "s_mov_b64 exec, %[sv]\n\ts_waitcnt lgkmcnt(0)"
-#define TILED_COMMIT_OPERANDS : [sv] "=&s"(sv), [lim] "+s"(lim) : [a] "v"(a), [a1] "v"(a + 65536u) : "vcc", "scc", "memory"
-
-__device__ __forceinline__ void tiled_commit(double* tile, int n, bool ring_after) {
-    typedef __attribute__((address_space(3))) char lds_char;
-    const unsigned base = (unsigned)(uintptr_t)(lds_char*)tile;
-    const unsigned a = base + threadIdx.x * 16u;
-    int lim = (int)(base + (unsigned)n * 8u);
-    uint64_t sv;
-    if (ring_after)
-        asm volatile(TILED_COMMIT_ASM("16") TILED_COMMIT_OPERANDS);
-    else
-        asm volatile(TILED_COMMIT_ASM("0") TILED_COMMIT_OPERANDS);
-}
-
-#define ACC_TILED_PARAMS                                                                                                          \
-    const uint32_t* __restrict__ sroff, const double* __restrict__ sx, const int64_t* __restrict__ cstart,                            \
-        const uint8_t* __restrict__ cnt, int T, int NB, int64_t nwb, const double* __restrict__ F, int k, int TR, int64_t nrow,       \
-        int tiles_per_range, double* __restrict__ Bout, int64_t ncol, int KS, int ldf, int ldb, int64_t slab,                        \
-        const int32_t* __restrict__ perm, int range_fastest, const uint16_t* __restrict__ gtab, int tail_wg0, int tail_R,            \
-        double* __restrict__ tail_part, int64_t tail_slab
-#define ACC_TILED_ARGS \
-    sroff, sx, cstart, cnt, T, NB, nwb, F, k, TR, nrow, tiles_per_range, Bout, ncol, KS, ldf, ldb, slab, perm, range_fastest, gtab, \
-        tail_wg0, tail_R, tail_part, tail_slab
-template <int NSL>
-__device__ __forceinline__ void acc_tiled_body(ACC_TILED_PARAMS) {
-    asm volatile("" ::: "v255");
-    extern __shared__ __attribute__((aligned(16))) char smem[];
-    double* tile = reinterpret_cast<double*>(smem);
-    const int lane = threadIdx.x & 63;
-    const int wave = __builtin_amdgcn_readfirstlane((int)(threadIdx.x >> 6));
-    unsigned bx = blockIdx.x, by = blockIdx.y;
-    if (range_fastest) {
-        const unsigned unit = blockIdx.x + gridDim.x * blockIdx.y, nranges = gridDim.y;
-        bx = unit / nranges;
-        by = unit - bx * nranges;
-    }
-    unsigned nry = gridDim.y;
-    bool tail_piece = false;
-    if (tail_R > 1 && (int)bx >= tail_wg0) {
-        const unsigned u = bx - (unsigned)tail_wg0;
-        bx = (unsigned)tail_wg0 + u / (unsigned)tail_R;
-        by = u % (unsigned)tail_R;
-        nry = (unsigned)tail_R;
-        tail_piece = true;
-    }
-    const int64_t wb = (int64_t)bx * TILED_NW + wave;
-    const int t0 = (int)(((int64_t)by * T) / nry);
-    const int t1 = (int)((((int64_t)by + 1) * T) / nry);
-    const int D = TR >> 1;
-    const int b0 = 2 * t0, b1 = 2 * t1 < NB ? 2 * t1 : NB;
-    const bool wact = wb < nwb;
-    typedef __attribute__((address_space(3))) char lds_char;
-    constexpr int LMASK = NSL == 4 ? 15 : 31;
-    const unsigned lane16 = (unsigned)(uintptr_t)(lds_char*)smem + (lane & LMASK) * 16;
-    const unsigned slot = NSL == 2 ? (unsigned)((lane >> 5) * 32 + (lane & 15)) : (unsigned)lane;
-    const unsigned voff4 = slot * 4, voff8 = slot * 8;
-    constexpr unsigned LAP_R = (NSL == 4 ? 256u : 128u) * 8u;
-    const unsigned pfl = (unsigned)lane * (LAP_R / 64u) + (unsigned)ACC_TILED_PF_LAPS * LAP_R;
-
-    asm volatile(ACC_TILED_ZERO_ASM ::: "memory");
-
-    uint64_t rp = 0, xp = 0;
-    int phase = 0;
-    int64_t pos_next = 0;
-    if (wact) {
-        const int64_t pos = cstart[wb * NB + b0];
-        pos_next = cstart[wb * NB + b0 + 1];
-        const uint64_t r_ = reinterpret_cast<uint64_t>(sroff + pos), x_ = reinterpret_cast<uint64_t>(sx + pos);
-        rp = ((uint64_t)(uint32_t)__builtin_amdgcn_readfirstlane((unsigned)(r_ >> 32)) << 32) | (uint32_t)__builtin_amdgcn_readfirstlane((unsigned)r_);
-        xp = ((uint64_t)(uint32_t)__builtin_amdgcn_readfirstlane((unsigned)(x_ >> 32)) << 32) | (uint32_t)__builtin_amdgcn_readfirstlane((unsigned)x_);
-        if constexpr (NSL == 4)
-            asm volatile(ACC_TILED4_RING_FILL_ASM : [rp] "+s"(rp), [xp] "+s"(xp) : [voff4] "v"(voff4), [voff8] "v"(voff8) : ACC_TILED_CLOBBERS);
-        else
-            asm volatile(ACC_TILED2_RING_FILL_ASM : [rp] "+s"(rp), [xp] "+s"(xp) : [voff4] "v"(voff4), [voff8] "v"(voff8) : ACC_TILED_CLOBBERS);
-    }
-    if constexpr (NSL == 4) {
-        for (int e = (int)threadIdx.x; e < TILED_LDS_BYTES / 8; e += 64 * TILED_NW) tile[e] = 0.0;
-    }
-
-    const bool pf = NSL == 2 && KS == k && ldf == k;
-    auto block_rows = [&](int j) { const int64_t row0 = (int64_t)j * D; return (int)(nrow - row0 < D ? nrow - row0 : D); };
-    int64_t pos_cur = wact ? cstart[wb * NB + b0] : 0;
-    for (int b = b0; b < b1; ++b) {
-        const int nsets = (int)((pos_next - pos_cur) >> 6);
-        const int64_t pos_chunk = pos_cur;
-        pos_cur = pos_next;
-        if (wact && b + 1 < b1) pos_next = cstart[wb * NB + b + 2];
-
-        if (pf) {
-            if (b == b0) {
-#pragma clang loop unroll(disable)
-                for (int j = b; j <= b + 1 && j < b1; ++j) {
-                    tiled_issue(F + (int64_t)j * D * ldf, block_rows(j) * k);
-                    tiled_commit(tile + (j & 1) * D * KS, block_rows(j) * k, false);
-                }
-                __syncthreads();
-            }
-            if (b + 2 < b1) tiled_issue(F + (int64_t)(b + 2) * D * ldf, block_rows(b + 2) * k);
-        } else {
-#pragma clang loop unroll(disable)
-            for (int j = b == b0 ? b : b + 1; j <= b + 1 && j < b1; ++j) {
-                const int64_t row0 = (int64_t)j * D;
-                tiled_stage<NSL>(tile + (j & 1) * D * KS, F + row0 * ldf, block_rows(j), k, KS, ldf, j == b || b != b0);
-            }
-            if (b == b0 || b + 1 < b1) {
-                __builtin_amdgcn_s_waitcnt(0x0F70);
-                __syncthreads();
-            }
-        }
-        if (wact && nsets > 0) {
-            const uint64_t t_ = reinterpret_cast<uint64_t>(gtab + pos_chunk / (4 * NSL));
-            const uint64_t tp = ((uint64_t)(uint32_t)__builtin_amdgcn_readfirstlane((unsigned)(t_ >> 32)) << 32) | (uint32_t)__builtin_amdgcn_readfirstlane((unsigned)t_);
-            if constexpr (NSL == 2)
-                asm volatile(ACC_TILED2_CHUNK_ASM
-                             : [rp] "+s"(rp), [xp] "+s"(xp), [phase] "+s"(phase)
-                             : [ns] "s"(2 * nsets), [tp] "s"(tp), [lane16] "v"(lane16), [voff4] "v"(voff4), [voff8] "v"(voff8), [pfl] "v"(pfl)
-                             : ACC_TILED_CHUNK_CLOBBERS);
-            else
-                asm volatile(ACC_TILED4_CHUNK_ASM
-                             : [rp] "+s"(rp), [xp] "+s"(xp), [phase] "+s"(phase)
-                             : [ns] "s"(nsets), [tp] "s"(tp), [lane16] "v"(lane16), [voff4] "v"(voff4), [voff8] "v"(voff8), [pfl] "v"(pfl)
-                             : ACC_TILED_CHUNK_CLOBBERS);
-        }
-        if (pf && b + 2 < b1) {
-            __syncthreads();
-            tiled_commit(tile + (b & 1) * D * KS, block_rows(b + 2) * k, wact && nsets >= 4);
-            __syncthreads();
-        }
-    }
-    asm volatile("s_waitcnt vmcnt(0)" ::: "memory");
-    if (wact) {
-        double* out = Bout + (size_t)by * (size_t)slab;
-        const int f = 2 * (lane & LMASK);
-        const int64_t tail_pos0 = (int64_t)tail_wg0 * TILED_NW * (TILED_NP * NSL);
-        for (int p = 0; p < TILED_NP; ++p) {
-            double v0, v1;
-            acc_load(4 * p, v0, v1);
-            const int h = NSL == 4 ? (lane >> 4) : (lane >> 5);
-            const int64_t col = tiled_slot_col(perm, ncol, wb, h, p, NSL);
-            if (col >= 0) {
-                if (tail_piece) {
-                    const int64_t pos = wb * (TILED_NP * NSL) + NSL * p + h;
-                    double* o = tail_part + (size_t)by * (size_t)tail_slab + (pos - tail_pos0) * k;
-                    if (f < k) o[f] = v0;
-                    if (f + 1 < k) o[f + 1] = v1;
-                } else {
-                    if (f < k) out[col * ldb + f] = v0;
-                    if (f + 1 < k) out[col * ldb + f + 1] = v1;
-                }
-            }
-        }
-    }
-}
-
 template <int NSL>
 __global__ __launch_bounds__(512) __attribute__((amdgpu_waves_per_eu(8, 8))) void acc_tiled_kernel(ACC_TILED_PARAMS) {
     acc_tiled_body<NSL>(ACC_TILED_ARGS);
@@ -735,14 +467,18 @@
     const int64_t tail_cols = tail ? (nwg_x - S.tail_wg0) * TILED_NW * S.CW : 0;
     const int64_t tail_slab = tail_cols * kf;
     const dim3 grid(tail ? (unsigned)(S.tail_wg0 + (nwg_x - S.tail_wg0) * S.tail_R) : (unsigned)nwg_x, (unsigned)S.R);
+#define K_ACC_TILED_LAUNCH_ARGS                                                                                                        \
+    S.roff, xvals ? xvals : S.x, S.cstart, S.cnt, S.T, S.NB, S.nwb, F, kf, S.TR, S.nrow, S.tiles_per_range, out, S.ncol, KS, ldf,       \
+        slabs ? kf : ldb, slabs ? n : 0, S.perm, S.range_fastest ? 1 : 0, S.gtab, tail ? (int)S.tail_wg0 : -1, tail ? S.tail_R : 1,     \
+        S.part, tail_slab
     auto launch = [&](auto nsl) {
-        acc_tiled_kernel<decltype(nsl)::value><<<grid, dim3(64 * TILED_NW), lds, s>>>(
-            S.roff, xvals ? xvals : S.x, S.cstart, S.cnt, S.T, S.NB, S.nwb, F, kf, S.TR, S.nrow, S.tiles_per_range, out, S.ncol, KS, ldf,
-            slabs ? kf : ldb, slabs ? n : 0, S.perm, S.range_fastest ? 1 : 0, S.gtab, tail ? (int)S.tail_wg0 : -1, tail ? S.tail_R : 1,
-            S.part, tail_slab);
+        acc_tiled_kernel<decltype(nsl)::value><<<grid, dim3(64 * TILED_NW), lds, s>>>(K_ACC_TILED_LAUNCH_ARGS);
     };
-    if (S.NSL == 4) launch(std::integral_constant<int, 4>());
+    const bool late = S.NSL == 2 && KS == kf && ldf == kf && !getenv("SGL_TILED_NO_LATE_PIECES");
+    if (late) SGLCHK(k_acc_tiled_late_launch(s, grid, lds, K_ACC_TILED_LAUNCH_ARGS));
+    else if (S.NSL == 4) launch(std::integral_constant<int, 4>());
     else launch(std::integral_constant<int, 2>());
+#undef K_ACC_TILED_LAUNCH_ARGS
     HIPCHK(hipGetLastError());
     if (tail) {
         const int64_t pos0 = S.tail_wg0 * TILED_NW * S.CW;
diff --git a/singlet_amd/csrc/kernels_tiled_late.hip b/singlet_amd/csrc/kernels_tiled_late.hip
--- /dev/null
+++ b/singlet_amd/csrc/kernels_tiled_late.hip
@@ -0,0 +1,13 @@
+#include "sgl_internal.h"
+#include "acc_tiled_late_gen.inc"
+#include "acc_tiled_body.h"
+
+__global__ __launch_bounds__(512) __attribute__((amdgpu_waves_per_eu(8, 8), amdgpu_num_vgpr(12))) void acc_tiled_late_kernel(ACC_TILED_PARAMS) {
+    acc_tiled_body<2>(ACC_TILED_ARGS);
+}
+
+int k_acc_tiled_late_launch(hipStream_t s, dim3 grid, size_t lds, ACC_TILED_PARAMS) {
+    SGLCHK(sgl_allow_dynamic_lds<&acc_tiled_late_kernel>(TILED_LDS_BYTES + 512));
+    acc_tiled_late_kernel<<<grid, dim3(64 * TILED_NW), lds, s>>>(ACC_TILED_ARGS);
+    return SGL_OK;
+}
```

Measured after the change: 42.07. Within noise of the previous version (-0.1%).
